# RapidAI/RapidDoc

Measured on AMD Instinct MI355X. Metric: pages/sec (layout+OCR det/rec), higher is better.
Workload: dtype f32

## Files before the change

### include/rapiddoc_mi355.h

```cpp
#ifndef RAPIDDOC_MI355_H
#define RAPIDDOC_MI355_H

#include <stddef.h>
#include <stdint.h>

#ifdef __cplusplus
extern "C" {
#endif

typedef struct rd_handle rd_handle;

#define RD_REC_UNFUSED_CTC 1
#define RD_REC_WANT_SOFTMAX 2
#define RD_REC_WANT_LOGITS 4
#define RD_REC_WANT_NECK 64

const char* rd_version(void);
rd_handle* rd_create(int device_id, const char* model_kind);
const char* rd_create_error(void);
void rd_destroy(rd_handle* h);
const char* rd_last_error(rd_handle* h);

int rd_load_weights(rd_handle* h, const void* safetensors_image, size_t nbytes);

int rd_query_workspace(rd_handle* h, int B, int H, int W, int flags, size_t* ws_bytes);

int rd_det_forward(rd_handle* h, const float* x_nchw_dev, int B, int H, int W, float* prob_b1hw_dev, void* ws_dev,
                   size_t ws_bytes, void* stream);
#define RD_DET_WANT_NECK 1
int rd_det_forward_ex(rd_handle* h, const float* x_nchw_dev, int B, int H, int W, float* prob_b1hw_dev, int flags, float* aux_dev,
                      void* ws_dev, size_t ws_bytes, void* stream);

int rd_rec_forward(rd_handle* h, const float* x_nchw_dev, int B, int W, int32_t* idx_bt_dev, float* prob_bt_dev,
                   float* full_btc_dev, int flags, void* ws_dev, size_t ws_bytes, void* stream);
int rd_rec_num_classes(rd_handle* h);
#define RD_REC_STAGE_BACKBONE 8
#define RD_REC_STAGE_TAIL 16
int rd_rec_token_dim(rd_handle* h);
int rd_rec_backbone_forward(rd_handle* h, const float* x_nchw_dev, int B, int W, float* tokens_btd_dev, void* ws_dev, size_t ws_bytes,
                            void* stream);
int rd_rec_tail_forward(rd_handle* h, const float* tokens_dev, int n_tokens, int n_lines, int max_tokens, const int32_t* seg_dev,
                        const int32_t* tokinfo_dev, int32_t* idx_dev, float* prob_dev, void* ws_dev, size_t ws_bytes, void* stream);
#define RD_REC_LINE_WIDTHS 32
int rd_rec_backbone_forward_lines(rd_handle* h, const float* x_nchw_dev, int B, int W, const int32_t* line_tab_dev, float* tokens_dev,
                                  void* ws_dev, size_t ws_bytes, void* stream);
int rd_rec_seq_len(int W);

int rd_backbone_forward(rd_handle* h, const float* x_nchw_dev, int B, int H, int W, float* const feats_dev[4],
                        void* ws_dev, size_t ws_bytes, void* stream);

int rd_formula_encoder_forward(rd_handle* h, const float* x_nchw_dev, int B, int C, int H, int W, float* enc_dev,
                               void* ws_dev, size_t ws_bytes, void* stream);

int rd_formula_decode(rd_handle* h, const float* enc_dev, int B, int S, int max_new_tokens, int64_t* ids_dev, int32_t* n_cols,
                      void* stream);
int rd_formula_max_new_tokens(rd_handle* h);

int rd_preproc_resize_norm(int device_id, const uint8_t* hwc_u8_dev, int H, int W, int OH, int OW, const float mean[3],
                           const float std[3], float scale, int interp, int swap_rb, float* out_chw_dev, void* stream);

int rd_preproc_resize_norm_batch(int device_id, const uint8_t* pages_u8_dev, int P, int H, int W, int OH, int OW, const float mean[3],
                                 const float std[3], float scale, int interp, int swap_rb, float* out_nchw_dev, void* stream);

#define RD_RESIZE_AA_MAX_SIDE 16384
int rd_preproc_resize_aa_norm(int device_id, const uint8_t* hwc_u8_dev, int H, int W, int OH, int OW, const float mean[3],
                              const float std[3], int swap_rb, float* out_chw_dev, uint8_t* out_u8_hwc_dev, void* stream);

typedef struct rd_crop_desc {
    int32_t page;
    int32_t out_w;
    float crop_w, crop_h;
    float m[9];
    int32_t rot90;
    int32_t pad_;
} rd_crop_desc;
int rd_crop_resize_norm_batch(int device_id, const uint8_t* pages_u8_dev, int P, int H, int W,
                              const rd_crop_desc* descs_dev, int n, int out_h, int out_w_padded, const float mean[3],
                              const float std[3], float scale, int swap_rb, float* out_nchw_dev, void* stream);

typedef struct rd_line_crop_desc {
    int32_t page;
    int32_t out_w;
    int32_t crop_w, crop_h;
    int32_t rot90;
    int32_t scratch_off;
    double m[9];
} rd_line_crop_desc;
int rd_line_crops_batch(int device_id, const uint8_t* pages_u8_dev, int P, int H, int W, const rd_line_crop_desc* descs_dev,
                        int n, int64_t max_crop_pixels, uint8_t* scratch_u8_dev, int out_h, int out_w_padded, int swap_rb,
                        float* out_nchw_dev, void* stream);

int rd_line_warp_batch(int device_id, const uint8_t* pages_u8_dev, int P, int H, int W, const rd_line_crop_desc* descs_dev, int n,
                       int64_t max_crop_pixels, uint8_t* scratch_u8_dev, void* stream);
int rd_line_resize_norm_batch(int device_id, const rd_line_crop_desc* descs_dev, int n, const uint8_t* scratch_u8_dev, int out_h,
                              int out_w_padded, int swap_rb, float* out_nchw_dev, void* stream);

#define RD_CLS_WANT_AUX 1
int rd_cls_forward(rd_handle* h, const float* x_nchw_dev, int B, int H, int W, float* prob_b2_dev, int flags, float* aux_dev, void* ws_dev,
                   size_t ws_bytes, void* stream);
int rd_table_encoder_forward(rd_handle* h, const float* x_nchw_dev, int B, int H, int W, float* memory_bt768_dev, void* ws_dev, size_t ws_bytes,
                             void* stream);
typedef struct {
    int32_t prefix_id, eos_id, pad_id, bbox_close_id, bbox_first_id, bbox_last_id;
} rd_table_decode_cfg;
int rd_table_decode(rd_handle* h, const float* memory_dev, int B, int S, int max_new_tokens, const rd_table_decode_cfg* cfg, int64_t* ids_dev,
                    int32_t* n_tokens, void* stream);
int rd_line_flip180_batch(int device_id, const rd_line_crop_desc* descs_dev, int n, const float* cls_prob_n2_dev, float thresh,
                          uint8_t* scratch_u8_dev, int32_t* flipped_out_dev, void* stream);

int rd_ctc_collapse(int device_id, const int32_t* idx_bt_dev, const float* prob_bt_dev, int B, int T, const uint8_t* char_table_dev,
                    int max_len, int n_classes, uint8_t* out_dev, int row_bytes, void* stream);
int rd_ctc_collapse_lines(int device_id, const int32_t* idx_dev, const float* prob_dev, int n_lines, const int32_t* seg_dev, int max_tokens,
                          const uint8_t* char_table_dev, int max_len, int n_classes, uint8_t* out_dev, int row_bytes, uint16_t* kept_cols_dev,
                          float* kept_conf_dev, void* stream);
int rd_ctc_rows_text(const uint8_t* rows_host, int n, int row_bytes, uint8_t* text_out, int64_t text_cap, int64_t* byte_off_out,
                     int32_t* n_chars_out, double* conf_out, double* conf3_out);

typedef struct rd_text_box {
    float pts[8];
    float score;
} rd_text_box;
int rd_db_postprocess(const float* prob_host, int B, int H, int W, const int32_t* src_hw, float thresh, float box_thresh,
                      float unclip_ratio, int use_dilation, int max_candidates, rd_text_box* out, int max_out,
                      int32_t* n_out, int n_threads);

size_t rd_db_boxes_workspace(int B, int H, int W, int max_runs, int max_candidates);
int rd_db_boxes_device(int device_id, const float* prob_dev, int B, int H, int W, const int32_t* src_hw_dev, float thresh, float box_thresh,
                       float unclip_ratio, int use_dilation, int max_candidates, int max_runs, void* ws_dev, size_t ws_bytes,
                       rd_text_box* out_dev, int max_out, int32_t* n_out_dev, void* stream);

int rd_text_boxes_order_merge(const rd_text_box* boxes, const int32_t* counts, int B, int max_in, float* quads_out, int32_t* n_out);

typedef struct rd_layout_post_cfg {
    int32_t n_classes;
    int32_t image_index, formula_index;
    int32_t thresh_is_dict;
    const float* thresh;
    int32_t layout_nms;
    int32_t merge_kind;
    const int8_t* merge_per_class;
    int32_t unclip_kind;
    const float* unclip;
    const uint8_t* unclip_present;
} rd_layout_post_cfg;
int rd_layout_postprocess(const float* boxes, int n, int ncol, int img_w, int img_h, const rd_layout_post_cfg* cfg,
                          float* out, int32_t* out_order, int32_t* n_out);
int rd_layout_postprocess_select(const float* boxes, int n, int ncol, int img_w, int img_h, const rd_layout_post_cfg* cfg,
                                 float* sel_boxes, int32_t* sel_src, int32_t* n_sel);

int rd_msdeform_attn(int device_id, const float* value, const int32_t* shapes, const int32_t* level_start, const float* loc, const float* attn,
                     float* out, int B, int S, int H, int D, int Q, int L, int P, void* stream);
int rd_topk_rows(int device_id, const float* scores, int rows, int n, int k, float* out_vals, int32_t* out_idx, void* stream);
size_t rd_encoder_layer_workspace(int M, int Dm, int F);
int rd_encoder_layer(int device_id, const float* x, const float* pos, int B, int T, int Dm, int heads, int F, int act, const float* in_w,
                     const float* in_b, const float* out_w, const float* out_b, const float* ln1_g, const float* ln1_b, const float* w1,
                     const float* b1, const float* w2, const float* b2, const float* ln2_g, const float* ln2_b, float eps, float* out, void* ws,
                     size_t ws_bytes, void* stream);

int rd_find_external_contours(const uint8_t* mask, int h, int w, int32_t* pts_out, int max_pts, int32_t* counts_out, int max_contours,
                              int32_t* n_contours, int32_t* n_pts);
double rd_contour_area(const int32_t* pts, int n);
double rd_arc_length(const int32_t* pts, int n, int closed);
int rd_approx_poly_dp(const int32_t* pts, int n, double epsilon, int closed, int32_t* out, int32_t* n_out);
int rd_min_area_rect_points(const float* pts, int n, float* out8);
double rd_polygon_area(const double* a, int na);
double rd_polygon_intersection_area(const double* a, int na, const double* b, int nb);
int rd_fill_poly(uint8_t* img, int h, int w, const int32_t* pts, int n, int value);

double rd_rec_chunk_cost(int n_lines, int wpad, int n_cu);
int rd_rec_plan_chunks(const int32_t* wpad_sorted, int n, int n_min, int n_max, int n_step, int n_cu, int32_t* sizes_out, int max_out,
                       int32_t* n_out);
int rd_rec_plan_lines(const double* ratios, const int64_t* order, int n, int rec_batch_num, int img_h, int img_w, int launch_multiple,
                      int n_min, int n_max, int n_step, int n_cu, int64_t* line_w_out, double* line_ratio_out, int32_t* sizes_out,
                      int32_t* launch_w_out, int max_out, int32_t* n_out);

int rd_set_precision(rd_handle* h, const char* mode);
int rd_range_status(rd_handle* h, void* stream);

int rd_plan_stats(rd_handle* h, uint64_t* plans_built, uint64_t* graph_captures, uint64_t* graph_replays);

int rd_set_profiling(rd_handle* h, int on);
const char* rd_profile_json(rd_handle* h);

#ifdef __cplusplus
}
#endif
#endif
```

### rapiddoc_amd/_lib.py

```python
from __future__ import annotations

import ctypes as C
from pathlib import Path

_PKG = Path(__file__).resolve().parent
LIB_PATH = _PKG / "librapiddoc_mi355.so"
_lib = None

SYMBOLS = {
    "rd_version": (C.c_char_p, []),
    "rd_create": (C.c_void_p, [C.c_int, C.c_char_p]),
    "rd_create_error": (C.c_char_p, []),
    "rd_destroy": (None, [C.c_void_p]),
    "rd_last_error": (C.c_char_p, [C.c_void_p]),
    "rd_load_weights": (C.c_int, [C.c_void_p, C.c_void_p, C.c_size_t]),
    "rd_query_workspace": (C.c_int, [C.c_void_p, C.c_int, C.c_int, C.c_int, C.c_int, C.POINTER(C.c_size_t)]),
    "rd_det_forward": (C.c_int, [C.c_void_p, C.c_void_p, C.c_int, C.c_int, C.c_int, C.c_void_p, C.c_void_p, C.c_size_t, C.c_void_p]),
    "rd_det_forward_ex": (C.c_int, [C.c_void_p, C.c_void_p, C.c_int, C.c_int, C.c_int, C.c_void_p, C.c_int, C.c_void_p, C.c_void_p, C.c_size_t, C.c_void_p]),
    "rd_rec_forward": (C.c_int, [C.c_void_p, C.c_void_p, C.c_int, C.c_int, C.c_void_p, C.c_void_p, C.c_void_p, C.c_int, C.c_void_p, C.c_size_t, C.c_void_p]),
    "rd_rec_num_classes": (C.c_int, [C.c_void_p]),
    "rd_rec_token_dim": (C.c_int, [C.c_void_p]),
    "rd_rec_backbone_forward": (C.c_int, [C.c_void_p, C.c_void_p, C.c_int, C.c_int, C.c_void_p, C.c_void_p, C.c_size_t, C.c_void_p]),
    "rd_rec_backbone_forward_lines": (C.c_int, [C.c_void_p, C.c_void_p, C.c_int, C.c_int, C.c_void_p, C.c_void_p, C.c_void_p, C.c_size_t, C.c_void_p]),
    "rd_rec_tail_forward": (C.c_int, [C.c_void_p, C.c_void_p, C.c_int, C.c_int, C.c_int, C.c_void_p, C.c_void_p, C.c_void_p, C.c_void_p,
                                      C.c_void_p, C.c_size_t, C.c_void_p]),
    "rd_rec_seq_len": (C.c_int, [C.c_int]),
    "rd_backbone_forward": (C.c_int, [C.c_void_p, C.c_void_p, C.c_int, C.c_int, C.c_int, C.POINTER(C.c_void_p), C.c_void_p, C.c_size_t, C.c_void_p]),
    "rd_formula_encoder_forward": (C.c_int, [C.c_void_p, C.c_void_p, C.c_int, C.c_int, C.c_int, C.c_int, C.c_void_p, C.c_void_p, C.c_size_t, C.c_void_p]),
    "rd_formula_decode": (C.c_int, [C.c_void_p, C.c_void_p, C.c_int, C.c_int, C.c_int, C.c_void_p, C.POINTER(C.c_int32), C.c_void_p]),
    "rd_formula_max_new_tokens": (C.c_int, [C.c_void_p]),
    "rd_preproc_resize_norm": (C.c_int, [C.c_int, C.c_void_p, C.c_int, C.c_int, C.c_int, C.c_int, C.POINTER(C.c_float), C.POINTER(C.c_float), C.c_float, C.c_int, C.c_int, C.c_void_p, C.c_void_p]),
    "rd_preproc_resize_norm_batch": (C.c_int, [C.c_int, C.c_void_p, C.c_int, C.c_int, C.c_int, C.c_int, C.c_int, C.POINTER(C.c_float), C.POINTER(C.c_float), C.c_float, C.c_int, C.c_int, C.c_void_p, C.c_void_p]),
    "rd_preproc_resize_aa_norm": (C.c_int, [C.c_int, C.c_void_p, C.c_int, C.c_int, C.c_int, C.c_int, C.POINTER(C.c_float), C.POINTER(C.c_float), C.c_int, C.c_void_p, C.c_void_p, C.c_void_p]),
    "rd_crop_resize_norm_batch": (C.c_int, [C.c_int, C.c_void_p, C.c_int, C.c_int, C.c_int, C.c_void_p, C.c_int, C.c_int, C.c_int, C.POINTER(C.c_float), C.POINTER(C.c_float), C.c_float, C.c_int, C.c_void_p, C.c_void_p]),
    "rd_line_crops_batch": (C.c_int, [C.c_int, C.c_void_p, C.c_int, C.c_int, C.c_int, C.c_void_p, C.c_int, C.c_int64, C.c_void_p, C.c_int, C.c_int, C.c_int, C.c_void_p, C.c_void_p]),
    "rd_line_warp_batch": (C.c_int, [C.c_int, C.c_void_p, C.c_int, C.c_int, C.c_int, C.c_void_p, C.c_int, C.c_int64, C.c_void_p, C.c_void_p]),
    "rd_line_resize_norm_batch": (C.c_int, [C.c_int, C.c_void_p, C.c_int, C.c_void_p, C.c_int, C.c_int, C.c_int, C.c_void_p, C.c_void_p]),
    "rd_cls_forward": (C.c_int, [C.c_void_p, C.c_void_p, C.c_int, C.c_int, C.c_int, C.c_void_p, C.c_int, C.c_void_p, C.c_void_p, C.c_size_t, C.c_void_p]),
    "rd_table_encoder_forward": (C.c_int, [C.c_void_p, C.c_void_p, C.c_int, C.c_int, C.c_int, C.c_void_p, C.c_void_p, C.c_size_t, C.c_void_p]),
    "rd_table_decode": (C.c_int, [C.c_void_p, C.c_void_p, C.c_int, C.c_int, C.c_int, C.c_void_p, C.c_void_p, C.c_void_p, C.c_void_p]),
    "rd_line_flip180_batch": (C.c_int, [C.c_int, C.c_void_p, C.c_int, C.c_void_p, C.c_float, C.c_void_p, C.c_void_p, C.c_void_p]),
    "rd_ctc_collapse": (C.c_int, [C.c_int, C.c_void_p, C.c_void_p, C.c_int, C.c_int, C.c_void_p, C.c_int, C.c_int, C.c_void_p, C.c_int, C.c_void_p]),
    "rd_ctc_collapse_lines": (C.c_int, [C.c_int, C.c_void_p, C.c_void_p, C.c_int, C.c_void_p, C.c_int, C.c_void_p, C.c_int, C.c_int, C.c_void_p, C.c_int, C.c_void_p, C.c_void_p,
                                        C.c_void_p]),
    "rd_db_postprocess": (C.c_int, [C.c_void_p, C.c_int, C.c_int, C.c_int, C.c_void_p, C.c_float, C.c_float, C.c_float, C.c_int, C.c_int, C.c_void_p, C.c_int, C.c_void_p, C.c_int]),
    "rd_db_boxes_workspace": (C.c_size_t, [C.c_int, C.c_int, C.c_int, C.c_int, C.c_int]),
    "rd_db_boxes_device": (C.c_int, [C.c_int, C.c_void_p, C.c_int, C.c_int, C.c_int, C.c_void_p, C.c_float, C.c_float, C.c_float, C.c_int, C.c_int,
                                     C.c_int, C.c_void_p, C.c_size_t, C.c_void_p, C.c_int, C.c_void_p, C.c_void_p]),
    "rd_rec_chunk_cost": (C.c_double, [C.c_int, C.c_int, C.c_int]),
    "rd_rec_plan_chunks": (C.c_int, [C.c_void_p, C.c_int, C.c_int, C.c_int, C.c_int, C.c_int, C.c_void_p, C.c_int, C.c_void_p]),
    "rd_rec_plan_lines": (C.c_int, [C.c_void_p, C.c_void_p] + [C.c_int] * 9 + [C.c_void_p] * 4 + [C.c_int, C.c_void_p]),
    "rd_text_boxes_order_merge": (C.c_int, [C.c_void_p, C.c_void_p, C.c_int, C.c_int, C.c_void_p, C.c_void_p]),
    "rd_ctc_rows_text": (C.c_int, [C.c_void_p, C.c_int, C.c_int, C.c_void_p, C.c_int64, C.c_void_p, C.c_void_p, C.c_void_p, C.c_void_p]),
    "rd_layout_postprocess": (C.c_int, [C.c_void_p, C.c_int, C.c_int, C.c_int, C.c_int, C.c_void_p, C.c_void_p, C.c_void_p, C.c_void_p]),
    "rd_layout_postprocess_select": (C.c_int, [C.c_void_p, C.c_int, C.c_int, C.c_int, C.c_int, C.c_void_p, C.c_void_p, C.c_void_p, C.c_void_p]),
    "rd_find_external_contours": (C.c_int, [C.c_void_p, C.c_int, C.c_int, C.c_void_p, C.c_int, C.c_void_p, C.c_int, C.c_void_p, C.c_void_p]),
    "rd_contour_area": (C.c_double, [C.c_void_p, C.c_int]),
    "rd_arc_length": (C.c_double, [C.c_void_p, C.c_int, C.c_int]),
    "rd_approx_poly_dp": (C.c_int, [C.c_void_p, C.c_int, C.c_double, C.c_int, C.c_void_p, C.c_void_p]),
    "rd_min_area_rect_points": (C.c_int, [C.c_void_p, C.c_int, C.c_void_p]),
    "rd_polygon_area": (C.c_double, [C.c_void_p, C.c_int]),
    "rd_polygon_intersection_area": (C.c_double, [C.c_void_p, C.c_int, C.c_void_p, C.c_int]),
    "rd_fill_poly": (C.c_int, [C.c_void_p, C.c_int, C.c_int, C.c_void_p, C.c_int, C.c_int]),
    "rd_msdeform_attn": (C.c_int, [C.c_int] + [C.c_void_p] * 6 + [C.c_int] * 7 + [C.c_void_p]),
    "rd_topk_rows": (C.c_int, [C.c_int, C.c_void_p, C.c_int, C.c_int, C.c_int, C.c_void_p, C.c_void_p, C.c_void_p]),
    "rd_encoder_layer_workspace": (C.c_size_t, [C.c_int, C.c_int, C.c_int]),
    "rd_encoder_layer": (C.c_int, [C.c_int, C.c_void_p, C.c_void_p] + [C.c_int] * 6 + [C.c_void_p] * 12 + [C.c_float, C.c_void_p, C.c_void_p, C.c_size_t, C.c_void_p]),
    "rd_set_precision": (C.c_int, [C.c_void_p, C.c_char_p]),
    "rd_range_status": (C.c_int, [C.c_void_p, C.c_void_p]),
    "rd_plan_stats": (C.c_int, [C.c_void_p, C.POINTER(C.c_uint64), C.POINTER(C.c_uint64), C.POINTER(C.c_uint64)]),
    "rd_set_profiling": (C.c_int, [C.c_void_p, C.c_int]),
    "rd_profile_json": (C.c_char_p, [C.c_void_p]),
}

_I, _P, _F = C.c_int, C.c_void_p, C.c_float
DEBUG_SYMBOLS = {
    "rd_debug_det_forward_stages": (_I, [_P, _P, _I, _I, _I, _P, _P, _P]),
    "rd_debug_cls_forward_stages": (_I, [_P, _P, _I, _I, _I, _P, _P, _P, _P]),
    "rd_debug_table_decode": (_I, [_P, _P, _I, _I, _I, _P] + [_P] * 7),
    "rd_debug_table_encoder_taps": (_I, [_P, _P, _I, _I, _I, _P, _P, _P]),
    "rd_debug_formula_decode": (_I, [_P, _P, _I, _I, _I, _P, C.POINTER(C.c_int32), _P, _P, _P]),
    "rd_debug_resize_aa_coeffs": (_I, [_I, _I, _P, _P, C.c_int64]),
    "rd_debug_time_mixer": (_F, [_I] * 4 + [_P] * 6),
    "rd_debug_time_gemm": (_F, [_I] * 5 + [_P] * 6),
    "rd_debug_gemm_h1": (_F, [_I] * 5 + [_P, _I, _P, _P, _P, _I, _P, _I, _P]),
    "rd_debug_seqconv": (_F, [_I] * 8 + [_P, _I, _P, _I, _P, _P, _P, _P, _I, _P]),
    "rd_debug_det_local": (_F, [_I] * 5 + [_P] * 5 + [_F, _P, C.POINTER(C.c_int)]),
    "rd_debug_conv": (_F, [_I] * 14 + [_P] * 8),
    "rd_debug_stem34": (_F, [_I] * 11 + [_P] * 7),
    "rd_debug_dwconv": (_F, [_I] * 8 + [_P] * 8),
    "rd_debug_lcv3_dw": (_F, [_I] * 9 + [_P] * 8),
    "rd_debug_dw5_strip": (_F, [_I] * 11 + [_P] * 7),
    "rd_debug_mv1e_pool": (_I, [_I] * 4 + [_P] * 3),
    "rd_debug_derived_tensor": (C.c_long, [C.c_char_p, C.c_char_p, C.c_size_t, C.c_char_p, _P, C.c_long]),
    "rd_debug_mbv3_dw": (_F, [_I] * 12 + [_P] * 4),
    "rd_debug_mbv3_block": (_F, [_I] * 14 + [_P] * 8),
    "rd_debug_mbv3_block_ok": (_I, [_I] * 12),
    "rd_debug_mbv3s_dw": (_F, [_I] * 13 + [_P] * 4),
    "rd_debug_mbv3s_block": (_F, [_I] * 15 + [_P] * 12),
    "rd_debug_lcv3_dw_det": (_F, [_I] * 10 + [_P] * 5),
    "rd_debug_lcv3_block": (_F, [_I] * 9 + [_P] * 9),
    "rd_debug_time_ctc": (_F, [_I] * 4 + [_P] * 7 + [_I, _P]),
    "rd_debug_attention": (_I, [_I] * 4 + [_F, _P, _P, _P, _I, _P]),
    "rd_debug_vit_attention": (_I, [_I] * 4 + [_F, _P, _P]),
    "rd_debug_attention_limits": (_I, [_I, _P, _P]),
    "rd_debug_layernorm": (_I, [_I, _I, _P, _I, _P, _I, _P, _P, _F]),
    "rd_debug_ctc_head": (_I, [_I] * 3 + [_P, _I] + [_P] * 6 + [_I, _P, _P]),
    "rd_debug_dec_gemv": (_I, [_I] * 4 + [_P] * 7),
    "rd_debug_dec_attention": (_I, [_I] * 4 + [_P, _P, _I, C.c_longlong] + [_P] * 5 + [_P, _I, _P, _P, _I, _P, _I]),
    "rd_debug_dec_select": (_I, [_I, _P, _I, _I, _I, _P, _I, _P, _I, _I] + [_P] * 6),
}


class NativeLibraryError(RuntimeError):
    pass


def load():
    global _lib
    if _lib is not None:
        return _lib
    if not LIB_PATH.exists():
        raise NativeLibraryError(
            f"{LIB_PATH} is missing - build it with `python -m rapiddoc_amd.build` (hipcc, gfx950). "
            "rapiddoc_amd has no CPU fallback.")
    import torch
    lib = C.CDLL(str(LIB_PATH))
    for name, (res, args) in {**SYMBOLS, **DEBUG_SYMBOLS}.items():
        fn = getattr(lib, name)
        fn.restype = res
        fn.argtypes = args
    _lib = lib
    return lib
```

### rapiddoc_amd/build.py

```python
from __future__ import annotations

import os
import shutil
import subprocess
import sys
from concurrent.futures import ThreadPoolExecutor
from pathlib import Path

PKG = Path(__file__).resolve().parent
CSRC = PKG / "csrc"
OUT = PKG / "librapiddoc_mi355.so"
SOURCES = ["kernels_conv.hip", "kernels_conv_h3.hip", "kernels_conv_direct_h3.hip", "kernels_conv3x3_h1.hip", "kernels_conv9x9_h1.hip", "kernels_stem34.hip", "kernels_rtdetr.hip", "kernels_conv_stream_h3.hip", "kernels_gemm_h3_dma.hip", "kernels_gemm_h1.hip", "kernels_misc.hip", "kernels_dw_lds.hip", "kernels_stem_fused.hip", "kernels_image.hip", "kernels_resize_aa.hip", "kernels_dbpost.hip", "kernels_attention_h3.hip", "kernels_seqconv.hip", "kernels_det_local.hip", "kernels_lcv3.hip", "kernels_lcv3_det.hip", "kernels_mv1e.hip", "kernels_mbv3.hip", "kernels_mbv3s.hip", "kernels_vit_attn.hip", "kernels_lcv3_block.hip", "kernels_ctc.hip", "kernels_mixer.hip", "kernels_mixer_h3.hip", "kernels_mixer_ws.hip", "kernels_mixer_res.hip", "formula_decoder.hip", "table_decoder.hip", "engine.cpp", "builder.cpp", "builder_mobile.cpp", "models.cpp", "api.cpp", "api_debug.cpp", "db_postprocess.cpp", "layout_postprocess.cpp", "polygon_ops.cpp", "rec_chunks.cpp", "host_stages.cpp"]
FLAGS = ["--offload-arch=gfx950", "-O3", "-std=c++17", "-fPIC", "-Wall", "-Wno-unused-function", "-x", "hip"]
FILE_FLAGS = {"kernels_mixer_ws.hip": ["-fno-slp-vectorize", "-DRD_GELU_SCALAR"], "kernels_gemm_h1.hip": ["-fno-slp-vectorize"],
              "kernels_stem_fused.hip": ["-fno-slp-vectorize"]}


def extra_flags_for(src: str) -> list:
    return list(FILE_FLAGS.get(Path(src).name, []))


def _hipcc() -> str:
    for cand in (os.environ.get("HIPCC"), shutil.which("hipcc"), "/opt/rocm/bin/hipcc"):
        if cand and Path(cand).exists():
            return cand
    raise RuntimeError("hipcc not found (ROCm 7.x required)")


def needs_build() -> bool:
    if not OUT.exists():
        return True
    t = OUT.stat().st_mtime
    deps = list(CSRC.glob("*")) + [PKG.parent / "include" / "rapiddoc_mi355.h", Path(__file__)]
    return any(d.stat().st_mtime > t for d in deps)


def build(force: bool = False, verbose: bool = True, extra_flags: tuple = (), out: Path = None) -> Path:
    variant = out is not None
    if not variant and not force and not needs_build():
        return OUT
    hipcc = _hipcc()
    objdir = PKG / "build" / (Path(out).stem if variant else "")
    objdir.mkdir(parents=True, exist_ok=True)
    OUT_ = Path(out) if variant else OUT

    def compile_one(src: str) -> Path:
        obj = objdir / (src + ".o")
        cmd = [hipcc, *FLAGS, *extra_flags_for(src), *extra_flags, "-c", str(CSRC / src), "-o", str(obj)]
        r = subprocess.run(cmd, capture_output=True, text=True)
        if r.returncode != 0:
            raise RuntimeError(f"hipcc failed for {src}:\n{r.stdout}\n{r.stderr}")
        if verbose and r.stderr.strip():
            print(r.stderr, file=sys.stderr)
        return obj

    with ThreadPoolExecutor(max_workers=min(8, len(SOURCES))) as ex:
        objs = list(ex.map(compile_one, SOURCES))
    tmp = OUT_.with_name(OUT_.name + f".tmp{os.getpid()}")
    cmd = [hipcc, "--offload-arch=gfx950", "-shared", "-fPIC", *map(str, objs), "-o", str(tmp)]
    r = subprocess.run(cmd, capture_output=True, text=True)
    if r.returncode != 0:
        tmp.unlink(missing_ok=True)
        raise RuntimeError(f"link failed:\n{r.stdout}\n{r.stderr}")
    os.replace(tmp, OUT_)
    if verbose:
        print(f"built {OUT_} ({OUT_.stat().st_size/1e6:.1f} MB)")
    return OUT_


if __name__ == "__main__":
    build(force="--force" in sys.argv)
```

### rapiddoc_amd/csrc/api.cpp

```cpp
#include <algorithm>
#include <mutex>
#include <string>

#include "api_handle.h"

static thread_local std::string g_create_err;

static bool is_family(const rd_handle* h, rd::ModelFamily f) { return h->eng && h->eng->model().family == f; }
static bool is_rec(const rd_handle* h) { return is_family(h, rd::ModelFamily::Recogniser); }
static bool is_det(const rd_handle* h) { return is_family(h, rd::ModelFamily::Detector); }

extern "C" {

const char* rd_version(void) { return "rapiddoc_mi355 0.3 (gfx950; fp32 results, split-fp16 + fp32 MFMA kernels)"; }

rd_handle* rd_create(int device_id, const char* model_kind) {
    try {
        if (!model_kind) throw rd::Error("model_kind is NULL");
        auto* h = new rd_handle();
        h->device = device_id;
        h->kind = model_kind;
        if (h->kind == "ppformulanet_head" || h->kind == "unitable_decoder") {
            int count = 0;
            if (hipGetDeviceCount(&count) != hipSuccess || count <= 0 || device_id < 0 || device_id >= count) {
                delete h;
                throw rd::Error("no HIP device available (MI355X required; there is no CPU fallback)");
            }
        } else {
            h->eng = new rd::Engine(device_id, model_kind);
        }
        g_create_err.clear();
        return h;
    } catch (const std::exception& e) {
        g_create_err = e.what();
        return nullptr;
    }
}
const char* rd_create_error(void) { return g_create_err.c_str(); }

void rd_destroy(rd_handle* h) {
    if (!h) return;
    delete h->eng;
    if (h->dec) rd::formula_decoder_destroy(h->dec);
    if (h->tdec) rd::table_decoder_destroy(h->tdec);
    delete h;
}
const char* rd_last_error(rd_handle* h) { return h ? h->err.c_str() : "null handle"; }

int rd_load_weights(rd_handle* h, const void* img, size_t nbytes) {
    return guarded(h, [&] {
        if (h->kind == "ppformulanet_head") {
            RD_CHECK(!h->dec, "weights already loaded for this handle");
            h->dec = rd::formula_decoder_create(h->device, img, nbytes);
        } else if (h->kind == "unitable_decoder") {
            RD_CHECK(!h->tdec, "weights already loaded for this handle");
            h->tdec = rd::table_decoder_create(h->device, img, nbytes);
        } else {
            h->eng->load_weights(img, nbytes);
        }
    });
}

int rd_query_workspace(rd_handle* h, int B, int H, int W, int flags, size_t* ws_bytes) {
    return guarded(h, [&] {
        RD_CHECK(ws_bytes, "ws_bytes is NULL");
        RD_CHECK(h->eng, "this model kind owns its workspace");
        if (is_rec(h) && !(flags & rd::REC_STAGE_TAIL)) H = 48;
        *ws_bytes = h->eng->workspace_bytes(B, H, W, flags);
    });
}

int rd_det_forward(rd_handle* h, const float* x, int B, int H, int W, float* prob, void* ws, size_t ws_bytes, void* stream) {
    return guarded(h, [&] {
        RD_CHECK(is_det(h), "handle is not a detector (ppocrv6_det / ppocrv5_det_server / ppocrv5_det_mobile / ppocrv3_det_mobile) model");
        RD_CHECK(x && prob && B > 0, "null input/output");
        h->eng->run(B, H, W, 0, {(void*)x, (void*)prob}, ws, ws_bytes, (hipStream_t)stream);
    });
}

int rd_det_forward_ex(rd_handle* h, const float* x, int B, int H, int W, float* prob, int flags, float* aux, void* ws, size_t ws_bytes,
                      void* stream) {
    return guarded(h, [&] {
        RD_CHECK(is_det(h), "handle is not a detector (ppocrv6_det / ppocrv5_det_server / ppocrv5_det_mobile / ppocrv3_det_mobile) model");
        RD_CHECK(x && prob && B > 0, "null input/output");
        RD_CHECK((flags & ~RD_DET_WANT_NECK) == 0, "rd_det_forward_ex: unknown flag");
        if (flags & RD_DET_WANT_NECK) {
            RD_CHECK(h->eng->model().det_want_neck,
                     "RD_DET_WANT_NECK is offered by ppocrv5_det_server, ppocrv5_det_mobile and ppocrv3_det_mobile only");
            RD_CHECK(aux, "aux_dev is NULL");
        }
        h->eng->run(B, H, W, flags, {(void*)x, (void*)prob, (void*)aux}, ws, ws_bytes, (hipStream_t)stream);
    });
}

int rd_cls_forward(rd_handle* h, const float* x, int B, int H, int W, float* prob, int flags, float* aux, void* ws, size_t ws_bytes, void* stream) {
    return guarded(h, [&] {
        RD_CHECK(h->eng && h->eng->kind() == "ppocr_cls_mobile", "handle is not a text-line classifier (ppocr_cls_mobile) model");
        RD_CHECK(x && prob && B > 0, "null input/output");
        RD_CHECK((flags & ~RD_CLS_WANT_AUX) == 0, "rd_cls_forward: unknown flag");
        RD_CHECK(!(flags & RD_CLS_WANT_AUX) || aux, "aux_dev is NULL");
        h->eng->run(B, H, W, flags, {(void*)x, (void*)prob, (void*)aux}, ws, ws_bytes, (hipStream_t)stream);
    });
}

int rd_table_encoder_forward(rd_handle* h, const float* x, int B, int H, int W, float* memory, void* ws, size_t ws_bytes, void* stream) {
    return guarded(h, [&] {
        RD_CHECK(h->eng && h->eng->kind() == "unitable_encoder", "handle is not a table-structure encoder (unitable_encoder) model");
        RD_CHECK(x && memory && B > 0, "null input/output");
        h->eng->run(B, H, W, 0, {(void*)x, (void*)memory}, ws, ws_bytes, (hipStream_t)stream);
    });
}


int rd_table_decode(rd_handle* h, const float* memory, int B, int S, int max_new_tokens, const rd_table_decode_cfg* cfg, int64_t* ids, int32_t* n_tokens,
                    void* stream) {
    return guarded(h, [&] {
        RD_CHECK(h->kind == "unitable_decoder" && h->tdec, "handle is not a loaded table-structure decoder (unitable_decoder)");
        int c[6];
        table_cfg6(cfg, c);
        rd::table_decoder_decode(h->tdec, memory, B, S, max_new_tokens, c, (long long*)ids, (int*)n_tokens, (hipStream_t)stream, nullptr, nullptr, nullptr,
                                 nullptr, nullptr);
    });
}

int rd_line_flip180_batch(int device_id, const rd_line_crop_desc* descs, int n, const float* cls_prob, float thresh, uint8_t* scratch,
                          int32_t* flipped_out, void* stream) {
    if (!descs || !cls_prob || !scratch || !flipped_out || n < 0) return 1;
    if (hipSetDevice(device_id) != hipSuccess) return 1;
    if (rd::launch_line_flip180(reinterpret_cast<const rd::LineCropDesc*>(descs), n, cls_prob, thresh, scratch, flipped_out, (hipStream_t)stream) != 0) return 1;
    return hipGetLastError() == hipSuccess ? 0 : 1;
}

int rd_rec_forward(rd_handle* h, const float* x, int B, int W, int32_t* idx, float* prob, float* full, int flags, void* ws,
                   size_t ws_bytes, void* stream) {
    return guarded(h, [&] {
        RD_CHECK(is_rec(h), "handle is not a recogniser (ppocrv6_rec / ppocrv5_rec_server / ppocrv5_rec_mobile / ppocr_rec_mv1e) model");
        RD_CHECK(x && idx && prob && B > 0, "null input/output");
        if (flags & (RD_REC_WANT_SOFTMAX | RD_REC_WANT_LOGITS | RD_REC_WANT_NECK)) RD_CHECK(full, "full_btc_dev is NULL");
        RD_CHECK(!((flags & RD_REC_WANT_SOFTMAX) && (flags & RD_REC_WANT_LOGITS)), "choose softmax OR logits");
        RD_CHECK(!(flags & RD_REC_WANT_NECK) || flags == RD_REC_WANT_NECK, "RD_REC_WANT_NECK goes with no other flag");
        h->eng->run(B, 48, W, flags, {(void*)x, (void*)idx, (void*)prob, (void*)full}, ws, ws_bytes, (hipStream_t)stream);
    });
}
int rd_rec_token_dim(rd_handle* h) { return (h && is_rec(h)) ? h->eng->rec_token_dim() : -1; }
int rd_rec_backbone_forward(rd_handle* h, const float* x, int B, int W, float* tokens, void* ws, size_t ws_bytes, void* stream) {
    return guarded(h, [&] {
        RD_CHECK(is_rec(h), "handle is not a recogniser (ppocrv6_rec / ppocrv5_rec_server / ppocrv5_rec_mobile / ppocr_rec_mv1e) model");
        RD_CHECK(x && tokens && B > 0, "null input/output");
        h->eng->run(B, 48, W, rd::REC_STAGE_BACKBONE, {(void*)x, (void*)tokens}, ws, ws_bytes, (hipStream_t)stream);
    });
}
int rd_rec_backbone_forward_lines(rd_handle* h, const float* x, int B, int W, const int32_t* line_tab, float* tokens, void* ws, size_t ws_bytes,
                                  void* stream) {
    return guarded(h, [&] {
        RD_CHECK(is_rec(h), "handle is not a ppocrv6_rec / ppocrv5_rec_mobile / ppocr_rec_mv1e model");
        RD_CHECK(h->eng->model().rec_line_widths, "rd_rec_backbone_forward_lines: per-line widths inside one backbone launch are out of scope for " +
                                                      h->eng->kind() + " (run the backbone stage once per padded width)");
        RD_CHECK(x && tokens && line_tab && B > 0, "null input/output");
        h->eng->run(B, 48, W, rd::REC_STAGE_BACKBONE | rd::REC_LINE_WIDTHS, {(void*)x, (void*)tokens, (void*)line_tab}, ws, ws_bytes,
                    (hipStream_t)stream);
    });
}
int rd_rec_tail_forward(rd_handle* h, const float* tokens, int n_tokens, int n_lines, int max_tokens, const int32_t* seg,
                        const int32_t* tokinfo, int32_t* idx, float* prob, void* ws, size_t ws_bytes, void* stream) {
    return guarded(h, [&] {
        RD_CHECK(is_rec(h), "handle is not a recogniser (ppocrv6_rec / ppocrv5_rec_server / ppocrv5_rec_mobile / ppocr_rec_mv1e) model");
        RD_CHECK(tokens && seg && tokinfo && idx && prob && n_tokens > 0 && n_lines > 0 && max_tokens > 0, "null input/output");
        h->eng->run(n_lines, max_tokens, n_tokens, rd::REC_STAGE_TAIL,
                    {(void*)tokens, (void*)idx, (void*)prob, nullptr, (void*)seg, (void*)tokinfo}, ws, ws_bytes, (hipStream_t)stream);
    });
}
int rd_rec_seq_len(int W) {
    if (W < 16) return 0;
    const int w1 = (W - 1) / 2 + 1, w2 = (w1 - 1) / 2 + 1;
    return (w2 - 2) / 2 + 1;
}
int rd_rec_num_classes(rd_handle* h) { return (h && h->eng) ? h->eng->n_classes() : -1; }

int rd_backbone_forward(rd_handle* h, const float* x, int B, int H, int W, float* const feats[4], void* ws, size_t ws_bytes,
                        void* stream) {
    return guarded(h, [&] {
        RD_CHECK(h->eng && h->eng->kind() == "pphgnetv2_b4", "handle is not a pphgnetv2_b4 model");
        RD_CHECK(x && feats && feats[0] && feats[1] && feats[2] && feats[3], "null input/output");
        h->eng->run(B, H, W, 0, {(void*)x, (void*)feats[0], (void*)feats[1], (void*)feats[2], (void*)feats[3]}, ws, ws_bytes,
                    (hipStream_t)stream);
    });
}

int rd_formula_encoder_forward(rd_handle* h, const float* x, int B, int C, int H, int W, float* enc, void* ws, size_t ws_bytes,
                               void* stream) {
    return guarded(h, [&] {
        RD_CHECK(h->eng && h->eng->kind() == "pphgnetv2_b6_formula", "handle is not a pphgnetv2_b6_formula model");
        RD_CHECK(x && enc && B > 0 && (C == 1 || C == 3), "null input/output or channel count not 1/3");
        h->eng->run(B, H, W, C == 1 ? 1 : 0, {(void*)x, (void*)enc}, ws, ws_bytes, (hipStream_t)stream);
    });
}

int rd_formula_decode(rd_handle* h, const float* enc, int B, int S, int max_new_tokens, int64_t* ids, int32_t* n_cols, void* stream) {
    return guarded(h, [&] {
        RD_CHECK(h->kind == "ppformulanet_head" && h->dec, "handle is not a loaded ppformulanet_head model");
        RD_CHECK(enc && ids && n_cols, "null input/output");
        *n_cols = rd::formula_decoder_decode(h->dec, enc, B, S, max_new_tokens, reinterpret_cast<long long*>(ids), (hipStream_t)stream, nullptr,
                                             nullptr);
    });
}
int rd_formula_max_new_tokens(rd_handle* h) { return (h && h->dec) ? rd::formula_decoder_max_new(h->dec) : -1; }

int rd_preproc_resize_norm(int device_id, const uint8_t* src, int H, int W, int OH, int OW, const float mean[3],
                           const float std[3], float scale, int interp, int swap_rb, float* out, void* stream) {
    if (!src || !out || H <= 0 || W <= 0 || OH <= 0 || OW <= 0 || (interp != 1 && interp != 2)) return 1;
    if (hipSetDevice(device_id) != hipSuccess) return 1;
    rd::PreprocParams p{};
    p.src = src; p.H = H; p.W = W; p.dst = out; p.OH = OH; p.OW = OW;
    for (int i = 0; i < 3; ++i) { p.mean[i] = mean ? mean[i] : 0.f; p.inv_std[i] = 1.f / (std ? std[i] : 1.f); }
    p.scale = scale; p.interp = interp; p.swap_rb = swap_rb;
    rd::launch_preproc_resize_norm(p, (hipStream_t)stream);
    return hipGetLastError() == hipSuccess ? 0 : 1;
}

int rd_preproc_resize_norm_batch(int device_id, const uint8_t* src, int P, int H, int W, int OH, int OW, const float mean[3],
                                 const float std[3], float scale, int interp, int swap_rb, float* out, void* stream) {
    if (!src || !out || P <= 0 || P > 65535 || H <= 0 || W <= 0 || OH <= 0 || OW <= 0 || (interp != 1 && interp != 2)) return 1;
    if (hipSetDevice(device_id) != hipSuccess) return 1;
    rd::PreprocParams p{};
    p.src = src; p.H = H; p.W = W; p.dst = out; p.OH = OH; p.OW = OW;
    for (int i = 0; i < 3; ++i) { p.mean[i] = mean ? mean[i] : 0.f; p.inv_std[i] = 1.f / (std ? std[i] : 1.f); }
    p.scale = scale; p.interp = interp; p.swap_rb = swap_rb;
    p.batch = P; p.src_stride = (size_t)H * W * 3; p.dst_stride = (size_t)3 * OH * OW;
    rd::launch_preproc_resize_norm(p, (hipStream_t)stream);
    return hipGetLastError() == hipSuccess ? 0 : 1;
}

int rd_preproc_resize_aa_norm(int device_id, const uint8_t* src, int H, int W, int OH, int OW, const float mean[3], const float std[3],
                              int swap_rb, float* out, uint8_t* out_u8, void* stream) {
    std::string err;
    const int rc = rd::launch_resize_aa_norm(device_id, src, H, W, OH, OW, mean, std, swap_rb, out, out_u8, (hipStream_t)stream, err);
    if (rc != 0) g_create_err = err;
    return rc;
}

int rd_crop_resize_norm_batch(int device_id, const uint8_t* pages, int P, int H, int W, const rd_crop_desc* descs, int n,
                              int out_h, int out_w_padded, const float mean[3], const float std[3], float scale, int swap_rb,
                              float* out, void* stream) {
    static_assert(sizeof(rd_crop_desc) == sizeof(rd::CropDesc), "rd_crop_desc layout");
    if (!pages || !descs || !out || P <= 0 || n < 0 || out_h <= 0 || out_w_padded <= 0) return 1;
    if (hipSetDevice(device_id) != hipSuccess) return 1;
    rd::CropBatchParams p{};
    p.pages = pages; p.H = H; p.W = W; p.page_stride = (size_t)H * W * 3;
    p.descs = reinterpret_cast<const rd::CropDesc*>(descs); p.n = n;
    p.dst = out; p.OH = out_h; p.OWp = out_w_padded;
    for (int i = 0; i < 3; ++i) { p.mean[i] = mean ? mean[i] : 0.f; p.inv_std[i] = 1.f / (std ? std[i] : 1.f); }
    p.scale = scale; p.swap_rb = swap_rb;
    rd::launch_crop_resize_norm_batch(p, (hipStream_t)stream);
    return hipGetLastError() == hipSuccess ? 0 : 1;
}

int rd_line_crops_batch(int device_id, const uint8_t* pages, int P, int H, int W, const rd_line_crop_desc* descs, int n,
                        int64_t max_crop_pixels, uint8_t* scratch, int out_h, int out_w_padded, int swap_rb, float* out, void* stream) {
    static_assert(sizeof(rd_line_crop_desc) == sizeof(rd::LineCropDesc), "rd_line_crop_desc layout");
    if (!pages || !descs || !out || !scratch || P <= 0 || n < 0 || out_h <= 0 || out_w_padded <= 0 || max_crop_pixels <= 0) return 1;
    if (hipSetDevice(device_id) != hipSuccess) return 1;
    rd::LineCropParams p{};
    p.pages = pages; p.H = H; p.W = W; p.page_stride = (size_t)H * W * 3;
    p.descs = reinterpret_cast<const rd::LineCropDesc*>(descs); p.n = n;
    p.scratch = scratch; p.max_crop_pixels = (long)max_crop_pixels;
    p.dst = out; p.OH = out_h; p.OWp = out_w_padded; p.swap_rb = swap_rb;
    if (rd::launch_line_crops(p, (hipStream_t)stream) != 0) return 1;
    return hipGetLastError() == hipSuccess ? 0 : 1;
}

int rd_line_warp_batch(int device_id, const uint8_t* pages, int P, int H, int W, const rd_line_crop_desc* descs, int n,
                       int64_t max_crop_pixels, uint8_t* scratch, void* stream) {
    if (!pages || !descs || !scratch || P <= 0 || n < 0 || max_crop_pixels <= 0) return 1;
    if (hipSetDevice(device_id) != hipSuccess) return 1;
    rd::LineCropParams p{};
    p.pages = pages; p.H = H; p.W = W; p.page_stride = (size_t)H * W * 3;
    p.descs = reinterpret_cast<const rd::LineCropDesc*>(descs); p.n = n;
    p.scratch = scratch; p.max_crop_pixels = (long)max_crop_pixels;
    if (rd::launch_line_warp(p, (hipStream_t)stream) != 0) return 1;
    return hipGetLastError() == hipSuccess ? 0 : 1;
}
int rd_line_resize_norm_batch(int device_id, const rd_line_crop_desc* descs, int n, const uint8_t* scratch, int out_h, int out_w_padded,
                              int swap_rb, float* out, void* stream) {
    if (!descs || !scratch || !out || n < 0 || out_h <= 0 || out_w_padded <= 0) return 1;
    if (hipSetDevice(device_id) != hipSuccess) return 1;
    rd::LineCropParams p{};
    p.descs = reinterpret_cast<const rd::LineCropDesc*>(descs); p.n = n;
    p.scratch = const_cast<uint8_t*>(scratch);
    p.dst = out; p.OH = out_h; p.OWp = out_w_padded; p.swap_rb = swap_rb;
    if (rd::launch_line_resize_norm(p, (hipStream_t)stream) != 0) return 1;
    return hipGetLastError() == hipSuccess ? 0 : 1;
}

int rd_ctc_collapse(int device_id, const int32_t* idx, const float* prob, int B, int T, const uint8_t* ctab, int max_len, int n_classes,
                    uint8_t* out, int row_bytes, void* stream) {
    if (!idx || !prob || !ctab || !out || B < 0 || T <= 0 || max_len <= 0 || n_classes <= 0) return 1;
    if (hipSetDevice(device_id) != hipSuccess) return 1;
    if (rd::launch_ctc_collapse(idx, prob, B, T, nullptr, ctab, max_len, n_classes, out, row_bytes, nullptr, nullptr, (hipStream_t)stream) != 0) return 1;
    return hipGetLastError() == hipSuccess ? 0 : 1;
}

int rd_ctc_collapse_lines(int device_id, const int32_t* idx, const float* prob, int n_lines, const int32_t* seg, int max_tokens,
                          const uint8_t* ctab, int max_len, int n_classes, uint8_t* out, int row_bytes, uint16_t* kept_cols, float* kept_conf,
                          void* stream) {
    if (!idx || !prob || !seg || !ctab || !out || n_lines < 0 || max_tokens <= 0 || max_len <= 0 || n_classes <= 0) return 1;
    if (hipSetDevice(device_id) != hipSuccess) return 1;
    if (rd::launch_ctc_collapse(idx, prob, n_lines, max_tokens, seg, ctab, max_len, n_classes, out, row_bytes, kept_cols, kept_conf,
                                (hipStream_t)stream) != 0)
        return 1;
    return hipGetLastError() == hipSuccess ? 0 : 1;
}

int rd_msdeform_attn(int device_id, const float* value, const int32_t* shapes, const int32_t* level_start, const float* loc, const float* attn,
                     float* out, int B, int S, int H, int D, int Q, int L, int P, void* stream) {
    if (!value || !shapes || !level_start || !loc || !attn || !out || B < 0 || S <= 0 || H <= 0 || D <= 0 || Q < 0 || L <= 0 || P <= 0 || H * D > 1024)
        return 1;
    if (hipSetDevice(device_id) != hipSuccess) return 1;
    rd::launch_msdeform_attn(value, shapes, level_start, loc, attn, out, B, S, H, D, Q, L, P, (hipStream_t)stream);
    return hipGetLastError() == hipSuccess ? 0 : 1;
}

int rd_topk_rows(int device_id, const float* scores, int rows, int n, int k, float* out_vals, int32_t* out_idx, void* stream) {
    if (!scores || !out_vals || !out_idx || rows < 0 || n <= 0 || k <= 0 || k > 1024 || k > n) return 1;
    if (hipSetDevice(device_id) != hipSuccess) return 1;
    rd::launch_topk_rows(scores, rows, n, k, out_vals, out_idx, (hipStream_t)stream);
    return hipGetLastError() == hipSuccess ? 0 : 1;
}

size_t rd_encoder_layer_workspace(int M, int Dm, int F) {
    if (M <= 0 || Dm <= 0 || F <= 0) return 0;
    return ((size_t)M * Dm * 3  + (size_t)M * 3 * Dm  + (size_t)M * F) * sizeof(float);
}

int rd_encoder_layer(int device_id, const float* x, const float* pos, int B, int T, int Dm, int heads, int F, int act, const float* in_w,
                     const float* in_b, const float* out_w, const float* out_b, const float* ln1_g, const float* ln1_b, const float* w1,
                     const float* b1, const float* w2, const float* b2, const float* ln2_g, const float* ln2_b, float eps, float* out, void* ws,
                     size_t ws_bytes, void* stream) {
    const int M = B * T;
    if (!x || !in_w || !out_w || !w1 || !w2 || !ln1_g || !ln1_b || !ln2_g || !ln2_b || !out || !ws || B <= 0 || T <= 0 || heads <= 0 ||
        Dm % heads != 0 || Dm % 4 != 0 || F % 4 != 0 || ws_bytes < rd_encoder_layer_workspace(M, Dm, F))
        return 1;
    const int hd = Dm / heads;
    if (hd != 16 && hd != 32) return 1;
    if (hipSetDevice(device_id) != hipSuccess) return 1;
    hipStream_t s = (hipStream_t)stream;
    float* xp = (float*)ws;
    float* att = xp + (size_t)M * Dm;
    float* y1 = att + (size_t)M * Dm;
    float* qkv = y1 + (size_t)M * Dm;
    float* ff = qkv + (size_t)M * 3 * Dm;
    auto gemm = [&](const float* a, int K, const float* w, const float* b, int N, float* y, int yld, int a_act, const float* res) {
        rd::ConvParams p{};
        p.x = a; p.xld = K; p.N = 1; p.H = 1; p.W = M; p.Cin = K;
        p.w = w; p.bias = b; p.y = y; p.yld = yld; p.OH = 1; p.OW = M; p.Cout = N;
        p.KH = p.KW = p.SH = p.SW = 1;
        p.res = res; p.rld = N;
        p.act = a_act; p.out_mode = rd::OUT_NHWC;
        p.M = M; p.K = K; p.Ng = N;
        rd::launch_conv_igemm(p, s);
    };
    try {
        const float* qk_in = x;
        if (pos) {
            rd::launch_add(x, Dm, pos, Dm, xp, Dm, M, Dm, s);
            qk_in = xp;
        }
        gemm(qk_in, Dm, in_w, in_b, 2 * Dm, qkv, 3 * Dm, rd::ACT_NONE, nullptr);
        gemm(x, Dm, in_w + (size_t)2 * Dm * Dm, in_b ? in_b + 2 * Dm : nullptr, Dm, qkv + 2 * Dm, 3 * Dm, rd::ACT_NONE, nullptr);
        rd::launch_attention(qkv, att, B, T, heads, hd, 1.0f / std::sqrt((float)hd), s);
        gemm(att, Dm, out_w, out_b, Dm, xp, Dm, rd::ACT_NONE, x);
        rd::launch_layernorm(xp, Dm, y1, Dm, ln1_g, ln1_b, M, Dm, eps, s);
        gemm(y1, Dm, w1, b1, F, ff, F, act, nullptr);
        gemm(ff, F, w2, b2, Dm, xp, Dm, rd::ACT_NONE, y1);
        rd::launch_layernorm(xp, Dm, out, Dm, ln2_g, ln2_b, M, Dm, eps, s);
    } catch (...) {
        return 1;
    }
    return hipGetLastError() == hipSuccess ? 0 : 1;
}

size_t rd_db_boxes_workspace(int B, int H, int W, int max_runs, int max_candidates) {
    (void)W;
    if (B <= 0 || H <= 0 || max_runs <= 0 || max_candidates <= 0) return 0;
    return rd::db_boxes_workspace_bytes(B, H, max_runs, max_candidates);
}
int rd_db_boxes_device(int device_id, const float* prob, int B, int H, int W, const int32_t* src_hw_dev, float thresh, float box_thresh,
                       float unclip_ratio, int use_dilation, int max_candidates, int max_runs, void* ws, size_t ws_bytes, rd_text_box* out,
                       int max_out, int32_t* n_out, void* stream) {
    if (!prob || !src_hw_dev || !ws || !out || !n_out || B < 0 || H <= 0 || W <= 0) return 1;
    if (hipSetDevice(device_id) != hipSuccess) return 1;
    if (rd::launch_db_boxes(prob, B, H, W, src_hw_dev, thresh, box_thresh, unclip_ratio, use_dilation, max_candidates, max_runs, ws, ws_bytes,
                            out, max_out, n_out, (hipStream_t)stream) != 0)
        return 1;
    return hipGetLastError() == hipSuccess ? 0 : 1;
}

int rd_set_precision(rd_handle* h, const char* mode) {
    return guarded(h, [&] {
        RD_CHECK(h->eng, "precision modes apply to the network engines");
        const std::string m = mode ? mode : "";
        RD_CHECK(m == "auto" || m == "fp32" || m == "h3", "precision must be auto, fp32 or h3");
        h->eng->set_precision(m == "h3" ? rd::Engine::PREC_H3 : m == "fp32" ? rd::Engine::PREC_FP32 : rd::Engine::PREC_AUTO);
    });
}
int rd_range_status(rd_handle* h, void* stream) {
    int out = 0;
    const int rc = guarded(h, [&] { if (h->eng) out = h->eng->take_range_flag((hipStream_t)stream); });
    return rc != 0 ? -1 : out;
}

int rd_plan_stats(rd_handle* h, uint64_t* plans_built, uint64_t* graph_captures, uint64_t* graph_replays) {
    if (!h || !h->eng) return 1;
    if (plans_built) *plans_built = h->eng->plans_built();
    if (graph_captures) *graph_captures = h->eng->graph_captures();
    if (graph_replays) *graph_replays = h->eng->graph_replays();
    return 0;
}

int rd_set_profiling(rd_handle* h, int on) {
    return guarded(h, [&] { if (h->eng) h->eng->set_profiling(on != 0); });
}
const char* rd_profile_json(rd_handle* h) {
    if (!h || !h->eng) return "[]";
    h->prof = h->eng->profile_json();
    return h->prof.c_str();
}

}
```

### rapiddoc_amd/csrc/host_stages.cpp

```cpp
#include <algorithm>
#include <charconv>
#include <cstdint>
#include <cstring>
#include <vector>

#include "../../include/rapiddoc_mi355.h"

#pragma clang fp contract(off)

namespace {

struct Quad {
    float p[8];
};
struct BBox {
    float x0, y0, x1, y1;
};

bool quad_is_tilted(const Quad& q) {
    const float height = ((q.p[7] - q.p[1]) + (q.p[5] - q.p[3])) / 2.0f;
    const float diag = q.p[5] - q.p[1];
    return !(0.8f * height <= diag && diag <= 1.2f * height);
}

bool y_overlap_exceeds(const BBox& a, const BBox& b, float thr) {
    const float d = std::min(a.y1, b.y1) - std::max(a.y0, b.y0);
    const float ov = d > 0.0f ? d : 0.0f;
    const float mh = std::min(a.y1 - a.y0, b.y1 - b.y0);
    return mh > 0.0f ? (ov / mh) > thr : false;
}

void put_bbox(const BBox& b, float* o) {
    o[0] = b.x0; o[1] = b.y0; o[2] = b.x1; o[3] = b.y0; o[4] = b.x1; o[5] = b.y1; o[6] = b.x0; o[7] = b.y1;
}

int order_merge_page(const rd_text_box* in, int k, float* out) {
    std::vector<Quad> q((size_t)k);
    for (int i = 0; i < k; ++i)
        for (int c = 0; c < 8; ++c) q[i].p[c] = (float)(int32_t)in[i].pts[c];
    std::stable_sort(q.begin(), q.end(), [](const Quad& a, const Quad& b) { return a.p[1] < b.p[1] || (a.p[1] == b.p[1] && a.p[0] < b.p[0]); });
    for (int i = 0; i + 1 < k; ++i)
        for (int j = i; j >= 0; --j) {
            const float dy = q[j + 1].p[1] - q[j].p[1];
            if ((dy < 0.0f ? -dy : dy) < 10.0f && q[j + 1].p[0] < q[j].p[0]) std::swap(q[j], q[j + 1]);
            else break;
        }
    std::vector<BBox> flat;
    std::vector<int> tilted;
    flat.reserve((size_t)k);
    for (int i = 0; i < k; ++i) {
        if (quad_is_tilted(q[i])) tilted.push_back(i);
        else flat.push_back({q[i].p[0], q[i].p[1], q[i].p[2], q[i].p[5]});
    }
    std::stable_sort(flat.begin(), flat.end(), [](const BBox& a, const BBox& b) { return a.y0 < b.y0; });
    int n = 0;
    std::vector<BBox> line, merged;
    const size_t nf = flat.size();
    for (size_t lo = 0; lo < nf;) {
        size_t hi = lo + 1;
        while (hi < nf && y_overlap_exceeds(flat[hi], flat[hi - 1], 0.6f)) ++hi;
        float x_min = flat[lo].x0, x_max = flat[lo].x1, y_min = flat[lo].y0, y_max = flat[lo].y1;
        for (size_t i = lo + 1; i < hi; ++i) {
            x_min = std::min(x_min, flat[i].x0); x_max = std::max(x_max, flat[i].x1);
            y_min = std::min(y_min, flat[i].y0); y_max = std::max(y_max, flat[i].y1);
        }
        if (x_max - x_min > (y_max - y_min) * 4.0f) {
            line.assign(flat.begin() + lo, flat.begin() + hi);
            std::stable_sort(line.begin(), line.end(), [](const BBox& a, const BBox& b) { return a.x0 < b.x0; });
            merged.clear();
            for (BBox b : line) {
                if (!merged.empty() && !(merged.back().x1 < b.x0)) {
                    const BBox m = merged.back();
                    merged.pop_back();
                    b = {std::min(m.x0, b.x0), std::min(m.y0, b.y0), std::max(m.x1, b.x1), std::max(m.y1, b.y1)};
                }
                merged.push_back(b);
            }
            for (const BBox& m : merged) put_bbox(m, out + 8 * (size_t)n++);
        } else {
            for (size_t i = lo; i < hi; ++i) put_bbox(flat[i], out + 8 * (size_t)n++);
        }
        lo = hi;
    }
    for (int i : tilted) std::memcpy(out + 8 * (size_t)n++, q[i].p, sizeof(q[i].p));
    return n;
}

}

extern "C" int rd_text_boxes_order_merge(const rd_text_box* boxes, const int32_t* counts, int B, int max_in, float* quads_out, int32_t* n_out) {
    if (B < 0 || max_in < 0 || (B > 0 && (!boxes || !counts || !quads_out || !n_out))) return 1;
    for (int b = 0; b < B; ++b)
        if (counts[b] < 0 || counts[b] > max_in) return 1;
    for (int b = 0; b < B; ++b)
        n_out[b] = order_merge_page(boxes + (size_t)b * max_in, counts[b], quads_out + (size_t)b * max_in * 8);
    return 0;
}

extern "C" int rd_ctc_rows_text(const uint8_t* rows, int n, int row_bytes, uint8_t* text_out, int64_t text_cap, int64_t* byte_off_out,
                                int32_t* n_chars_out, double* conf_out, double* conf3_out) {
    if (n < 0 || row_bytes < 16 || text_cap < 0 || !byte_off_out || (n > 0 && (!rows || !n_chars_out || !conf_out || !conf3_out))) return 1;
    int64_t pos = 0;
    byte_off_out[0] = 0;
    for (int b = 0; b < n; ++b) {
        const uint8_t* row = rows + (size_t)b * row_bytes;
        int32_t nbytes;
        float conf;
        std::memcpy(&nbytes, row, 4);
        std::memcpy(&conf, row + 4, 4);
        if (nbytes < 0 || nbytes > row_bytes - 16) return 1;
        if (pos + nbytes > text_cap || (nbytes > 0 && !text_out)) return 2;
        int32_t chars = 0;
        for (int32_t i = 0; i < nbytes; ++i) {
            const uint8_t c = row[16 + i];
            text_out[pos + i] = c;
            chars += (c & 0xC0) != 0x80;
        }
        pos += nbytes;
        byte_off_out[b + 1] = pos;
        n_chars_out[b] = chars;
        const double s = (double)conf;
        conf_out[b] = s;
        char buf[400];
        const auto w = std::to_chars(buf, buf + sizeof(buf), s, std::chars_format::fixed, 3);
        double r = s;
        if (w.ec == std::errc()) std::from_chars(buf, w.ptr, r);
        conf3_out[b] = r;
    }
    return 0;
}
```

### rapiddoc_amd/pipeline.py

```python
from __future__ import annotations

import os
import time
import ctypes as C
from concurrent.futures import ThreadPoolExecutor
from dataclasses import dataclass, field
from typing import Dict, List, Optional, Sequence, Tuple

import numpy as np
import torch

from . import _lib, ocr_host
from .engine import RdEngine, preproc_resize_norm, preproc_resize_norm_batch
from .rec_plan import (CLS_IMG_H, CLS_IMG_W, LINE_DTYPE, RecPlan, plan_rec,
                       quad_to_crop_matrix, quads_to_crop_matrices)

LAYOUT_SIZE = 800
DET_LIMIT = 960


class CropDesc(C.Structure):
    _fields_ = [("page", C.c_int32), ("out_w", C.c_int32), ("crop_w", C.c_float), ("crop_h", C.c_float),
                ("m", C.c_float * 9), ("rot90", C.c_int32), ("pad_", C.c_int32)]


def cls_flip_rule(prob: np.ndarray, thresh: float) -> np.ndarray:
    p = np.asarray(prob, dtype=np.float32).reshape(-1, 2)
    return (p[:, 1] > p[:, 0]) & (p[:, 1] >= np.float32(thresh))


def flip180(crop: np.ndarray) -> np.ndarray:
    return np.ascontiguousarray(np.asarray(crop)[::-1, ::-1])


CROP_DTYPE = np.dtype([("page", "<i4"), ("out_w", "<i4"), ("crop_w", "<f4"), ("crop_h", "<f4"), ("m", "<f4", (9,)),
                       ("rot90", "<i4"), ("pad_", "<i4")])
assert CROP_DTYPE.itemsize == C.sizeof(CropDesc)


def boxes_to_quads(boxes_xyxy: np.ndarray) -> np.ndarray:
    b = np.asarray(boxes_xyxy, dtype=np.float32).reshape(-1, 4)
    return np.stack([b[:, [0, 1]], b[:, [2, 1]], b[:, [2, 3]], b[:, [0, 3]]], axis=1)


@dataclass
class PageResult:
    lines: List[Tuple[np.ndarray, str, float]] = field(default_factory=list)
    layout_feats: Optional[List[torch.Tensor]] = None
    cls: Optional[List[Tuple[bool, int, float]]] = None


@dataclass(slots=True)
class _RecLaunch:
    x: Optional[torch.Tensor] = None
    event: Optional[torch.cuda.Event] = None
    done: Optional[torch.cuda.Event] = None
    idx: Optional[torch.Tensor] = None
    prob: Optional[torch.Tensor] = None
    rows: Optional[torch.Tensor] = None
    cols: Optional[Tuple[torch.Tensor, torch.Tensor]] = None
    cls_prob: Optional[torch.Tensor] = None
    cls_flip: Optional[torch.Tensor] = None


class PagePipeline:
    def __init__(self, states: Dict[str, object], device: int = 0, characters: Optional[Sequence[str]] = None,
                 rec_batch_num: Optional[int] = None, rec_width_multiple: int = 32, keep_feats: bool = False, n_rec_streams: int = 4,
                 rec_mode: Optional[str] = None, rec_chunking: Optional[str] = None, use_cls: bool = False, cls_thresh: float = 0.9):
        self.use_cls, self.cls_thresh = bool(use_cls), float(cls_thresh)
        if self.use_cls and "ppocr_cls_mobile" not in states:
            raise ValueError("use_cls=True needs the text-line classifier's weights: states['ppocr_cls_mobile'] (ch_ptocr_mobile_v2.0_cls_mobile)")
        if rec_mode is None:
            rec_mode = "strict" if rec_batch_num is None and rec_chunking is None else "throughput"
        if rec_mode not in ("strict", "throughput"):
            raise ValueError("rec_mode must be 'strict' or 'throughput'")
        if rec_chunking is None:
            rec_chunking = "adaptive" if rec_batch_num is None else "fixed"
        if rec_batch_num is None:
            rec_batch_num = 64
        if rec_chunking not in ("fixed", "adaptive"):
            raise ValueError("rec_chunking must be 'fixed' or 'adaptive'")
        self.rec_mode = rec_mode
        self.rec_chunking = rec_chunking
        if rec_mode == "strict":
            rec_batch_num, rec_width_multiple = 6, 1
        self.device = device
        self.tdev = torch.device("cuda", device)
        self.n_cu = int(torch.cuda.get_device_properties(self.tdev).multi_processor_count)
        det_kinds = [k for k in ("ppocrv6_det", "ppocrv5_det_server", "ppocrv5_det_mobile", "ppocrv3_det_mobile") if k in states]
        if len(det_kinds) != 1:
            raise ValueError("states must carry exactly one detector: 'ppocrv6_det' or 'ppocrv5_det_server' or 'ppocrv5_det_mobile' or 'ppocrv3_det_mobile'")
        self.det_kind = det_kinds[0]
        self.det = RdEngine(self.det_kind, device, guard="deferred", reuse_outputs=True).load_weights(states[self.det_kind])
        rec_kinds = [k for k in ("ppocrv6_rec", "ppocrv5_rec_server", "ppocrv5_rec_mobile", "ppocr_rec_mv1e") if k in states]
        if len(rec_kinds) != 1:
            raise ValueError("states must carry exactly one recogniser: 'ppocrv6_rec' or 'ppocrv5_rec_server' or 'ppocrv5_rec_mobile' or 'ppocr_rec_mv1e'")
        self.rec_kind = rec_kinds[0]
        self.rec_lines_in_launch = self.rec_kind in ("ppocrv6_rec", "ppocrv5_rec_mobile", "ppocr_rec_mv1e")
        self.rec_engines = [RdEngine(self.rec_kind, device, guard="deferred").load_weights(states[self.rec_kind]) for _ in range(max(1, n_rec_streams))]
        self.rec = self.rec_engines[0]
        self.rec_streams = [torch.cuda.Stream(device=self.tdev) for _ in self.rec_engines]
        self.rec_tail = RdEngine(self.rec_kind, device, guard="deferred").load_weights(states[self.rec_kind])
        self.cls_engines = ([RdEngine("ppocr_cls_mobile", device, guard="deferred").load_weights(states["ppocr_cls_mobile"]) for _ in self.rec_engines]
                            if self.use_cls else [])
        self.last_cls = None
        self.tail_stream = torch.cuda.Stream(device=self.tdev)
        self.layout_stream = torch.cuda.Stream(device=self.tdev)
        self.front_stream = torch.cuda.Stream(device=self.tdev)
        self._prefetched: Optional[dict] = None
        self._after_rec_enqueue = None
        self.prefetch_gate = float(os.environ.get("RD_PREFETCH_GATE", "1.0"))
        self.layout = RdEngine("pphgnetv2_b4", device, guard="deferred", reuse_outputs=True).load_weights(states["pphgnetv2_b4"]) if "pphgnetv2_b4" in states else None
        self._bufs: Dict[tuple, torch.Tensor] = {}
        ncls = self.rec.num_classes
        self.characters = list(characters) if characters is not None else ["blank"] + [chr(0x4E00 + i) for i in range(ncls - 2)] + [" "]
        assert len(self.characters) == ncls, (len(self.characters), ncls)
        self.rec_batch_num = rec_batch_num
        self.rec_width_multiple = rec_width_multiple
        self.keep_feats = keep_feats
        tab, self._ctc_max_len = ocr_host.char_table(self.characters)
        self._ctc_table = torch.from_numpy(tab).to(self.tdev)
        self.device_ctc = True
        self.device_db = True
        self.host_native = ocr_host.host_native_default()
        self.db_ws: dict = {}
        self.rec_two_stage = os.environ.get("RD_REC_TWO_STAGE", "1") != "0"
        self.rec_width_sync = None
        self._sync_this_call = True
        self._width_sync_cache = None
        self._width_sync_epoch, self._in_run_batch = 0, False
        self.keep_rec_inputs = False
        self.last_rec_batches: List[Tuple[np.ndarray, torch.Tensor, torch.Tensor, torch.Tensor]] = []
        self._lib = _lib.load()
        self.stats: Dict[str, float] = {}

    def _buf(self, role, numel: int, dtype=torch.float32) -> torch.Tensor:
        key = (role, dtype)
        t = self._bufs.get(key)
        if t is None or t.numel() < numel:
            t = self._bufs[key] = torch.empty(int(numel * 1.25) + 64, dtype=dtype, device=self.tdev)
        return t[:numel]

    def layout_preprocess(self, pages: torch.Tensor) -> torch.Tensor:
        P = pages.shape[0]
        out = self._buf("layout_x", P * 3 * LAYOUT_SIZE * LAYOUT_SIZE).view(P, 3, LAYOUT_SIZE, LAYOUT_SIZE)
        return preproc_resize_norm_batch(pages, (LAYOUT_SIZE, LAYOUT_SIZE), interp=2, out=out)

    def layout_forward(self, pages: torch.Tensor) -> List[torch.Tensor]:
        return self.layout.backbone_forward(self.layout_preprocess(pages))

    def det_preprocess(self, pages: torch.Tensor) -> Tuple[torch.Tensor, Tuple[int, int]]:
        P, H, W, _ = pages.shape
        bh, bw = -(-(H + 100) // 64) * 64, -(-(W + 100) // 64) * 64
        dh, dw = ocr_host.det_resize_shape(bh, bw, DET_LIMIT, "max")
        out = self._buf("det_x", P * 3 * dh * dw).view(P, 3, dh, dw)
        x = preproc_resize_norm_batch(pages, (dh, dw), mean=ocr_host.DET_MEAN, std=ocr_host.DET_STD, interp=1, swap_rb=True, out=out)
        return x, (dh, dw)

    def det_forward(self, pages: torch.Tensor) -> Tuple[torch.Tensor, Tuple[int, int]]:
        x, det_hw = self.det_preprocess(pages)
        return self.det.det_forward(x), det_hw

    def rec_forward_lines(self, pages: torch.Tensor, quads_per_page: Sequence[np.ndarray]):
        return self.rec_forward_sources([(pages, quads_per_page)])[0]

    def rec_forward_sources(self, sources: Sequence[Tuple[torch.Tensor, Sequence[np.ndarray]]],
                            image_keys: Optional[Sequence[Sequence[int]]] = None, want_words: bool = False,
                            pooled: bool = True):
        self._sync_this_call = bool(pooled)
        if not self._in_run_batch:
            self._width_sync_epoch += 1
        out = self._rec_forward_sources_once(sources, image_keys, want_words)
        for _ in range(3):
            if not any([e.check_range_and_fallback() for e in self.rec_engines + [self.rec_tail] + self.cls_engines]):
                break
            self.stats["range_fallbacks"] = self.stats.get("range_fallbacks", 0) + 1
            out = self._rec_forward_sources_once(sources, image_keys, want_words)
        return out

    def _synced_widths(self, sync, keys: np.ndarray, ratios: np.ndarray):
        sig = (self._width_sync_epoch, keys.tobytes(), ratios.tobytes())
        if self._width_sync_cache is not None and self._width_sync_cache[0] == sig:
            return self._width_sync_cache[1]
        res = sync(keys, ratios)
        self._width_sync_cache = (sig, res)
        return res

    def _collapse_home(self, name: str, n: int, T: int, call, *extra: torch.Tensor) -> List[torch.Tensor]:
        row_bytes = (16 + T * self._ctc_max_len + 15) // 16 * 16
        rows = torch.empty((n, row_bytes), dtype=torch.uint8, device=self.tdev)
        if call(rows.data_ptr(), row_bytes) != 0:
            raise RuntimeError(f"{name} failed")
        home = []
        for t in (rows,) + extra:
            h = torch.empty(t.shape, dtype=t.dtype, pin_memory=True)
            h.copy_(t, non_blocking=True)
            home.append(h)
        return home

    def _collapse_rows(self, idx: torch.Tensor, prob: torch.Tensor, nb: int, st, record: bool = True):
        rows = done = None
        with torch.cuda.stream(st):
            if self.device_ctc:
                T = idx.shape[1]
                rows, = self._collapse_home("rd_ctc_collapse", nb, T, lambda out, row_bytes: self._lib.rd_ctc_collapse(
                    self.device, idx.data_ptr(), prob.data_ptr(), nb, T, self._ctc_table.data_ptr(), self._ctc_max_len, len(self.characters),
                    out, row_bytes, st.cuda_stream))
            if record:
                done = torch.cuda.Event()
                done.record(st)
        return rows, done

    def _collapse_lines(self, idx_all: torch.Tensor, prob_all: torch.Tensor, tables: torch.Tensor, n_lines: int, max_tokens: int, st,
                        want_cols: bool = False):
        with torch.cuda.stream(st):
            cols = torch.empty((n_lines, max_tokens), dtype=torch.int16, device=self.tdev) if want_cols else None
            confs = torch.empty((n_lines, max_tokens), dtype=torch.float32, device=self.tdev) if want_cols else None
            rows, *cols_h = self._collapse_home("rd_ctc_collapse_lines", n_lines, max_tokens, lambda out, row_bytes: self._lib.rd_ctc_collapse_lines(
                self.device, idx_all.data_ptr(), prob_all.data_ptr(), n_lines, tables.data_ptr(), max_tokens, self._ctc_table.data_ptr(),
                self._ctc_max_len, len(self.characters), out, row_bytes, cols.data_ptr() if want_cols else None,
                confs.data_ptr() if want_cols else None, st.cuda_stream), *((cols, confs) if want_cols else ()))
            done = torch.cuda.Event()
            done.record(st)
        return rows, done, tuple(cols_h) if want_cols else None

    def _rec_forward_sources_once(self, sources, image_keys=None, want_words=False):
        t0 = time.perf_counter()
        if self.use_cls and want_words:
            raise ValueError("use_cls together with want_words: rapidocr defines no word-box mapping for lines turned by 180 degrees")
        self.last_cls = None
        for imgs, _quads in sources:
            assert imgs.is_cuda and imgs.dtype == torch.uint8 and imgs.dim() == 4 and imgs.is_contiguous()
        strict = self.rec_mode == "strict"
        sync = None
        if self.rec_width_sync is not None and strict and self.rec_two_stage and self._sync_this_call:
            sync = lambda keys, ratios: self._synced_widths(self.rec_width_sync, keys, ratios)
        plan = plan_rec([(imgs.shape[0], quads) for imgs, quads in sources], image_keys, strict=strict, two_stage=self.rec_two_stage,
                        lines_in_launch=self.rec_lines_in_launch, chunking=self.rec_chunking, rec_batch_num=self.rec_batch_num,
                        rec_width_multiple=self.rec_width_multiple, n_cu=self.n_cu, n_streams=len(self.rec_engines), use_cls=self.use_cls,
                        host_native=self.host_native, want_words=want_words, width_sync=sync)
        scatter = lambda per_line: self._scatter_texts(per_line, plan.src_of, plan.page_of, plan.n_img, plan.perm)
        cls_of: List[tuple] = [(False, 0, 0.0)] * plan.n_all
        if plan.n == 0:
            if self.use_cls and plan.n_all:
                self.last_cls = scatter(cls_of)
            return scatter([("", 0.0, None) if want_words else ("", 0.0)] * plan.n_all)
        if getattr(self, "_crop_scratch", None) is None or self._crop_scratch.numel() < plan.scratch_bytes:
            self._crop_scratch = torch.empty(int(plan.scratch_bytes * 1.25) + 1024, dtype=torch.uint8, device=sources[0][0].device)
        self.stats["t_descs_ms"] = (time.perf_counter() - t0) * 1e3
        main = torch.cuda.current_stream()
        launches = self._enqueue_rec(plan, sources, want_words)
        self.stats["t_rec_enqueue_ms"] = (time.perf_counter() - t0) * 1e3 - self.stats["t_descs_ms"]
        hook, self._after_rec_enqueue = self._after_rec_enqueue, None
        if hook is not None:
            t_h = time.perf_counter()
            S, nb = len(self.rec_engines), len(launches)
            m = max(1, min(nb, int(np.ceil(self.prefetch_gate * nb))))
            hook([l.event for l in launches[max(0, m - S): m]])
            self.stats["t_front_next_ms"] = (time.perf_counter() - t_h) * 1e3
        texts = self._decode_rec(plan, launches, want_words)
        for st in self.rec_streams + [self.tail_stream]:
            main.wait_stream(st)
        self.stats["rec_lines"] = plan.n
        self.stats["rec_batches"] = len(launches)
        self.last_pool_order = plan.perm
        if self.use_cls:
            ph = np.concatenate([l.cls_prob.numpy() for l in launches])
            fh = np.concatenate([l.cls_flip.numpy() for l in launches])
            for j, i in enumerate(plan.line_ids.tolist()):
                label = int(ph[j, 1] > ph[j, 0])
                cls_of[i] = (bool(fh[j]), label, float(ph[j, label]))
            self.last_cls = scatter(cls_of)
            self.last_cls_prob = (plan.line_ids, ph)
        return scatter(texts)

    def _enqueue_rec(self, plan: RecPlan, sources, want_words: bool) -> List[_RecLaunch]:
        dev, S, lib = sources[0][0].device, len(self.rec_engines), self._lib
        keep_inputs = self.keep_rec_inputs
        upload = lambda descs: torch.from_numpy(descs.view(np.uint8)).to(dev, non_blocking=True)
        descs_dev = upload(plan.descs)
        cls = None
        if self.use_cls:
            cls = (upload(plan.descs_cls), self._buf("cls_prob", 2 * plan.n).view(plan.n, 2), self._buf("cls_flip", plan.n, torch.int32),
                   torch.empty((plan.n, 2), dtype=torch.float32, pin_memory=True), torch.empty((plan.n,), dtype=torch.int32, pin_memory=True))
        descs_warp_dev = upload(plan.descs_warp) if plan.descs_warp is not None else descs_dev
        if keep_inputs:
            self.last_rec_descs = (plan.descs.copy(), np.asarray(plan.batch_base, dtype=np.int64), np.asarray(plan.starts, dtype=np.int64))
            self.last_cls_inputs = []
        main = torch.cuda.current_stream()
        ready = torch.cuda.Event()
        ready.record(main)
        tokens = linetab = tables = None
        if plan.two_stage:
            base = plan.group_base
            tokens = self._buf("rec_tokens", int(base[-1]) * self.rec.rec_token_dim).view(int(base[-1]), self.rec.rec_token_dim)
            for gi, lens in enumerate(plan.group_lens):
                tokens[int(base[gi]) + int(lens.sum()): int(base[gi + 1])].zero_()
            tables = [self.rec_tail.rec_tail_tables(lp, dev, out=self._buf(("tail_tab", gi), 2 * len(lp) + int(lp.sum()), torch.int32))
                      for gi, (lp, _t) in enumerate(plan.group_pad)]
            if plan.linetab is not None:
                tab_h = torch.from_numpy(plan.linetab).pin_memory()
                linetab = self._buf("rec_linetab", 4 * plan.n, torch.int32).view(plan.n, 4)
                linetab.copy_(tab_h, non_blocking=True)
                self._keep_linetab = tab_h
            ready.record(main)
            self.tail_stream.wait_event(ready)
        launches: List[_RecLaunch] = []
        for bi, (chunk, wpad) in enumerate(plan.batches):
            nb, pos = len(chunk), int(plan.starts[bi])
            k = bi % S
            st = self.rec_streams[k]
            if bi < S:
                st.wait_event(ready)
            with torch.cuda.stream(st):
                x = self._buf(("rec_x", k), nb * 3 * ocr_host.REC_IMG_H * wpad).view(nb, 3, ocr_host.REC_IMG_H, wpad)
                scratch = self._crop_scratch.data_ptr() + int(plan.batch_base[bi])
                for si, first, cnt, max_px in plan.warp_jobs[bi]:
                    imgs = sources[si][0]
                    rc = lib.rd_line_warp_batch(self.device, imgs.data_ptr(), imgs.shape[0], imgs.shape[1], imgs.shape[2],
                                                descs_warp_dev.data_ptr() + first * LINE_DTYPE.itemsize, cnt, max_px, scratch, st.cuda_stream)
                    if rc != 0:
                        raise RuntimeError("rd_line_warp_batch failed")
                launch = _RecLaunch()
                if cls is not None:
                    self._enqueue_cls(launch, cls, descs_dev, k, pos, nb, scratch, plan.line_ids[pos: pos + nb])
                rc = lib.rd_line_resize_norm_batch(self.device, descs_dev.data_ptr() + pos * LINE_DTYPE.itemsize, nb, scratch,
                                                   ocr_host.REC_IMG_H, wpad, 1, x.data_ptr(), st.cuda_stream)
                if rc != 0:
                    raise RuntimeError("rd_line_resize_norm_batch failed")
                if plan.lines_in_launch:
                    self.rec_engines[k].rec_backbone_forward_lines(x, linetab[pos: pos + nb], tokens)
                elif plan.two_stage:
                    self.rec_engines[k].rec_backbone_forward(x, tokens[plan.tok_lo[bi]: plan.tok_lo[bi] + nb * int(plan.seq_line[pos])])
                else:
                    launch.idx, launch.prob, _ = self.rec_engines[k].rec_forward(x)
                    launch.rows, launch.done = self._collapse_rows(launch.idx, launch.prob, nb, st)
                launch.event = launch.done
                if plan.two_stage:
                    launch.event = torch.cuda.Event()
                    launch.event.record(st)
                launch.x = x.clone() if keep_inputs else x
            launches.append(launch)
            if plan.two_stage and ((bi + 1) % S == 0 or bi + 1 == len(plan.batches)):
                self._enqueue_tail(plan, launches, bi // S, tokens, tables[bi // S], want_words)
        return launches

    def _enqueue_cls(self, launch: _RecLaunch, cls, descs_dev, k: int, pos: int, nb: int, scratch: int, line_ids: np.ndarray) -> None:
        descs_cls_dev, cls_prob, cls_flip, cls_prob_h, cls_flip_h = cls
        stream = torch.cuda.current_stream().cuda_stream
        sl = slice(pos, pos + nb)
        xc = self._buf(("cls_x", k), nb * 3 * CLS_IMG_H * CLS_IMG_W).view(nb, 3, CLS_IMG_H, CLS_IMG_W)
        rc = self._lib.rd_line_resize_norm_batch(self.device, descs_cls_dev.data_ptr() + pos * LINE_DTYPE.itemsize, nb, scratch,
                                                 CLS_IMG_H, CLS_IMG_W, 1, xc.data_ptr(), stream)
        if rc != 0:
            raise RuntimeError("rd_line_resize_norm_batch (classifier) failed")
        self.cls_engines[k].cls_forward(xc, out=cls_prob[sl])
        if self.keep_rec_inputs:
            self.last_cls_inputs.append((line_ids, xc.clone()))
        rc = self._lib.rd_line_flip180_batch(self.device, descs_dev.data_ptr() + pos * LINE_DTYPE.itemsize, nb, cls_prob[sl].data_ptr(),
                                             self.cls_thresh, scratch, cls_flip[sl].data_ptr(), stream)
        if rc != 0:
            raise RuntimeError("rd_line_flip180_batch failed")
        launch.cls_prob, launch.cls_flip = cls_prob_h[sl], cls_flip_h[sl]
        launch.cls_prob.copy_(cls_prob[sl], non_blocking=True)
        launch.cls_flip.copy_(cls_flip[sl], non_blocking=True)

    def _enqueue_tail(self, plan: RecPlan, launches: List[_RecLaunch], gi: int, tokens: torch.Tensor, tables: torch.Tensor, want_words: bool) -> None:
        grp = [launches[bi] for bi in plan.groups[gi]]
        t_lo, t_hi = int(plan.group_base[gi]), int(plan.group_base[gi + 1])
        lens_pad, max_tokens = plan.group_pad[gi]
        for launch in grp:
            self.tail_stream.wait_event(launch.event)
        with torch.cuda.stream(self.tail_stream):
            n_tok = t_hi - t_lo
            idx_all, prob_all = self.rec_tail.rec_tail_forward(
                tokens[t_lo:t_hi], lens_pad, tables, max_tokens=max_tokens,
                out=(self._buf(("tail_idx", gi), n_tok, torch.int32), self._buf(("tail_prob", gi), n_tok)))
        done = None
        if plan.lines_mode:
            last = grp[-1]
            last.rows, done, last.cols = self._collapse_lines(idx_all, prob_all, tables, len(plan.group_lens[gi]), max_tokens, self.tail_stream,
                                                              want_words)
            if self.keep_rec_inputs:
                with torch.cuda.stream(self.tail_stream):
                    last.idx, last.prob = idx_all.clone(), prob_all.clone()
        else:
            for bi, launch in zip(plan.groups[gi], grp):
                nb, t = len(plan.batches[bi][0]), int(plan.seq_line[int(plan.starts[bi])])
                lo = plan.tok_lo[bi] - t_lo
                launch.idx, launch.prob = idx_all[lo: lo + nb * t].view(nb, t), prob_all[lo: lo + nb * t].view(nb, t)
                launch.rows, ev = self._collapse_rows(launch.idx, launch.prob, nb, self.tail_stream, record=launch is grp[-1])
                done = ev or done
        for launch in grp:
            launch.done = done

    def _texts_from_rows(self, rows_np: np.ndarray, line_ids: np.ndarray, texts: list) -> None:
        if self.host_native:
            txt, _conf, conf3 = ocr_host.parse_ctc_rows_native(rows_np)
            for i, t, s in zip(line_ids.tolist(), txt, conf3):
                texts[i] = (t, s)
        else:
            for i, (t, s) in zip(line_ids.tolist(), ocr_host.parse_ctc_rows(rows_np)):
                texts[i] = (t, ocr_host.format_score(s))

    def _words_from_rows(self, plan: RecPlan, lo: int, rows_np: np.ndarray, cols, texts: list) -> None:
        n_kept = rows_np[:, 8:12].copy().view("<i4")[:, 0]
        cols_np, confs_np = cols[0].numpy(), cols[1].numpy()
        for j, (t, sc) in enumerate(ocr_host.parse_ctc_rows(rows_np)):
            i, k = int(plan.order_all[lo + j]), int(n_kept[j])
            words = {"cols": cols_np[j, :k].astype(np.int64).tolist(), "confs": confs_np[j, :k].astype(np.float64).tolist(),
                     "n_steps": int(plan.seq_line[lo + j]), "wh_ratio": float(plan.ratios[i]), "max_wh_ratio": float(plan.line_ratio[lo + j]),
                     "crop_hw": (int(plan.eff_h[i]), int(plan.eff_w[i]))}
            texts[int(plan.keep[i])] = (t, sc, words)

    def _decode_groups(self, plan: RecPlan, launches: List[_RecLaunch], want_words: bool, texts: list) -> list:
        ids, starts = plan.line_ids, plan.starts
        t_dec = 0.0
        for gi, grp in enumerate(plan.groups):
            tail = launches[grp[-1]]
            tail.done.synchronize()
            t1 = time.perf_counter()
            lo, hi = int(starts[grp[0]]), int(starts[grp[-1] + 1])
            if want_words:
                self._words_from_rows(plan, lo, tail.rows.numpy(), tail.cols, texts)
            else:
                self._texts_from_rows(tail.rows.numpy(), ids[lo:hi], texts)
            t_dec += time.perf_counter() - t1
            if tail.idx is not None:
                g0 = int(plan.group_base[gi])
                for bi in grp:
                    a, e = int(starts[bi]), int(starts[bi + 1])
                    sl = [(int(plan.first_tok[i]) - g0, int(plan.seq_line[i])) for i in range(a, e)]
                    self.last_rec_batches.append((ids[a:e], launches[bi].x, np.asarray(plan.line_w[a:e]),
                                                  [tail.idx[o: o + t] for o, t in sl], [tail.prob[o: o + t] for o, t in sl]))
        self.stats["t_decode_ms"] = t_dec * 1e3
        return texts

    def _decode_rec(self, plan: RecPlan, launches: List[_RecLaunch], want_words: bool) -> list:
        texts: List[tuple] = [("", 0.0, None) if want_words else ("", 0.0)] * plan.n_all
        ids, starts = plan.line_ids, plan.starts
        t_dec = 0.0
        if self.keep_rec_inputs:
            self.last_rec_crop_sizes = (plan.crop_w.astype(np.int64), plan.crop_h.astype(np.int64), plan.rot90, plan.keep)
        if self.keep_rec_inputs or plan.lines_mode:
            self.last_rec_batches = []
        if plan.lines_mode:
            return self._decode_groups(plan, launches, want_words, texts)
        for bi, launch in enumerate(launches):
            ids_b = ids[int(starts[bi]): int(starts[bi + 1])]
            if self.keep_rec_inputs:
                self.last_rec_batches.append((ids_b, launch.x, launch.idx, launch.prob))
            launch.done.synchronize()
            if launch.rows is not None:
                t1 = time.perf_counter()
                self._texts_from_rows(launch.rows.numpy(), ids_b, texts)
            else:
                idx_h, prob_h = launch.idx.cpu().numpy(), launch.prob.cpu().numpy()
                t1 = time.perf_counter()
                for i, (t, s) in zip(ids_b.tolist(), ocr_host.ctc_decode(idx_h, prob_h, self.characters)):
                    texts[i] = (t, ocr_host.format_score(s))
            t_dec += time.perf_counter() - t1
        self.stats["t_decode_ms"] = t_dec * 1e3
        return texts

    @staticmethod
    def _scatter_texts(texts, src_of, page_of, n_img, perm=None):
        if perm is not None:
            inv = np.argsort(perm, kind="stable")
            texts = [texts[i] for i in inv.tolist()]
            src_of, page_of = src_of[inv], page_of[inv]
        out = [[[] for _ in range(k)] for k in n_img]
        for t, si, pi in zip(texts, src_of.tolist(), page_of.tolist()):
            out[si][pi].append(t)
        return out

    def boxes_from_maps(self, maps_host: np.ndarray, page_hw: Tuple[int, int], box_thresh: float = 0.3,
                        unclip_ratio: float = 1.8) -> List[np.ndarray]:
        P = maps_host.shape[0]
        res = ocr_host.db_postprocess(maps_host, [page_hw] * P, thresh=0.3, box_thresh=box_thresh, unclip_ratio=unclip_ratio,
                                      raw=self.host_native)
        t0 = time.perf_counter()
        if self.host_native:
            out = ocr_host.order_merge_boxes_native(*res)
            self.stats["t_boxes_ms"] = (time.perf_counter() - t0) * 1e3
            return out
        out = []
        for boxes, _scores in res:
            if len(boxes) == 0:
                out.append(np.zeros((0, 4, 2), np.float32))
                continue
            b = ocr_host.sorted_boxes(boxes.astype(np.float32))
            b = ocr_host.merge_det_boxes(b)
            out.append(np.asarray(b, dtype=np.float32).reshape(-1, 4, 2))
        self.stats["t_boxes_ms"] = (time.perf_counter() - t0) * 1e3
        return out

    def boxes_from_maps_device(self, maps_dev: torch.Tensor, page_hw: Tuple[int, int], box_thresh: float = 0.3,
                               unclip_ratio: float = 1.8) -> List[np.ndarray]:
        P = maps_dev.shape[0]
        res = ocr_host.db_postprocess_device(maps_dev, [page_hw] * P, thresh=0.3, box_thresh=box_thresh, unclip_ratio=unclip_ratio,
                                             stats=self.stats, cache=self.db_ws, raw=self.host_native)
        t0 = time.perf_counter()
        if self.host_native:
            out = ocr_host.order_merge_boxes_native(*res)
            self.stats["t_boxes_ms"] = (time.perf_counter() - t0) * 1e3
            return out
        out = []
        for boxes, _scores in res:
            if len(boxes) == 0:
                out.append(np.zeros((0, 4, 2), np.float32))
                continue
            b = ocr_host.merge_det_boxes(ocr_host.sorted_boxes(boxes.astype(np.float32)))
            out.append(np.asarray(b, dtype=np.float32).reshape(-1, 4, 2))
        self.stats["t_boxes_ms"] = (time.perf_counter() - t0) * 1e3
        return out

    def _boxes_via_host_maps(self, src: torch.Tensor, page_hw: Tuple[int, int]) -> List[np.ndarray]:
        if getattr(self, "_maps_host", None) is None or self._maps_host.shape != src.shape:
            self._maps_host = torch.empty(src.shape, dtype=torch.float32, pin_memory=True)
        t0 = time.perf_counter()
        self._maps_host.copy_(src, non_blocking=True)
        torch.cuda.current_stream().synchronize()
        t1 = time.perf_counter()
        quads = self.boxes_from_maps(self._maps_host.numpy(), page_hw)
        self.stats["t_wait_maps_ms"] = (t1 - t0) * 1e3
        self.stats["t_db_post_ms"] = (time.perf_counter() - t1) * 1e3 - self.stats["t_boxes_ms"]
        return quads

    def run_batch(self, pages: torch.Tensor, quads_per_page: Optional[Sequence[np.ndarray]] = None,
                  det_maps_override: Optional[torch.Tensor] = None, prefetch: Optional[torch.Tensor] = None,
                  page_keys: Optional[Sequence[int]] = None) -> List[PageResult]:
        if isinstance(pages, np.ndarray) or not pages.is_cuda:
            src = torch.from_numpy(np.ascontiguousarray(pages)) if isinstance(pages, np.ndarray) else pages.contiguous()
            pages = src.to(self.tdev, non_blocking=src.is_pinned())
        self._page_keys = None if page_keys is None else [int(k) for k in page_keys]
        assert self._page_keys is None or len(self._page_keys) == pages.shape[0]
        if self.rec_width_sync is not None and page_keys is None and getattr(self.rec_width_sync, "world_size", 1) > 1:
            raise ValueError("rec_width_sync over more than one rank needs page_keys: the pages' positions in the GLOBAL page list")
        self._width_sync_epoch += 1
        self._in_run_batch = True
        try:
            return self._run_batch_guarded(pages, quads_per_page, det_maps_override, prefetch)
        finally:
            self._in_run_batch = False

    def _run_batch_guarded(self, pages, quads_per_page, det_maps_override, prefetch):
        results = self._run_batch_once(pages, quads_per_page, det_maps_override, prefetch)
        engines = [self.det] + ([self.layout] if self.layout is not None else [])
        if os.environ.get("RD_DEV_SKIP_RANGE_CHECK") == "1":
            engines = []
        if any([e.check_range_and_fallback() for e in engines]):
            self.stats["range_fallbacks"] = self.stats.get("range_fallbacks", 0) + 1
            self._prefetched = None
            results = self._run_batch_once(pages, quads_per_page, det_maps_override, prefetch)
        return results

    @staticmethod
    def _front_key(pages: torch.Tensor) -> tuple:
        return (pages.data_ptr(), tuple(pages.shape))

    def _front(self, pages: torch.Tensor, n_results: int, gate: Sequence[torch.cuda.Event] = ()) -> dict:
        cur = torch.cuda.current_stream()
        h = {"key": self._front_key(pages), "feats": None, "layout_done": None}
        self.front_stream.wait_stream(cur)
        for ev in gate:
            self.front_stream.wait_event(ev)
        with torch.cuda.stream(self.front_stream):
            h["prob_maps"], h["det_hw"] = self.det_forward(pages)
            h["det_done"] = torch.cuda.Event()
            h["det_done"].record(self.front_stream)
        if self.layout is not None:
            self.layout_stream.wait_event(h["det_done"])
            with torch.cuda.stream(self.layout_stream):
                feats = self.layout_forward(pages)
                if self.keep_feats:
                    h["feats"] = [[f[i].clone() for f in feats] for i in range(n_results)]
                h["layout_done"] = torch.cuda.Event()
                h["layout_done"].record(self.layout_stream)
        return h

    def _run_batch_once(self, pages: torch.Tensor, quads_per_page: Optional[Sequence[np.ndarray]] = None,
                        det_maps_override: Optional[torch.Tensor] = None, prefetch: Optional[torch.Tensor] = None) -> List[PageResult]:
        assert pages.is_cuda and pages.dtype == torch.uint8 and pages.dim() == 4
        P, H, W, _ = pages.shape
        results = [PageResult() for _ in range(P)]
        cur = torch.cuda.current_stream()
        h, self._prefetched = self._prefetched, None
        if h is None or h["key"] != self._front_key(pages):
            h = self._front(pages, P)
            self.stats["front_prefetched"] = 0.0
        else:
            self.stats["front_prefetched"] = 1.0
        cur.wait_event(h["det_done"])
        if self.rec_width_sync is not None and self.det.precision != "fp32" and os.environ.get("RD_DEV_SKIP_RANGE_CHECK") != "1":
            if self.det.check_range_and_fallback():
                self.stats["range_fallbacks"] = self.stats.get("range_fallbacks", 0) + 1
                h = self._front(pages, P)
                self.stats["front_prefetched"] = 0.0
                cur.wait_event(h["det_done"])
        prob_maps, det_hw = h["prob_maps"], h["det_hw"]
        self.last_det = (prob_maps, det_hw)
        if quads_per_page is None:
            src = det_maps_override if det_maps_override is not None else prob_maps
            quads_per_page = self.boxes_from_maps_device(src.contiguous(), (H, W)) if self.device_db else self._boxes_via_host_maps(src, (H, W))
        if prefetch is not None:
            assert prefetch.is_cuda and prefetch.dtype == torch.uint8 and prefetch.dim() == 4

            def front_next(gate):
                self._prefetched = self._front(prefetch, prefetch.shape[0], gate)
            self._after_rec_enqueue = front_next
        try:
            keys = getattr(self, "_page_keys", None)
            texts = self.rec_forward_sources([(pages, quads_per_page)], image_keys=None if keys is None else [keys])[0]
        except BaseException:
            self._after_rec_enqueue = None
            raise
        if self._after_rec_enqueue is not None:
            self._after_rec_enqueue = None
            front_next(())
        if h["layout_done"] is not None:
            cur.wait_event(h["layout_done"])
        for i in range(P):
            qs = np.asarray(quads_per_page[i], dtype=np.float32).reshape(-1, 4, 2)
            results[i].lines = [(qs[j], t, s) for j, (t, s) in enumerate(texts[i])]
            if h["feats"] is not None:
                results[i].layout_feats = h["feats"][i]
            if self.use_cls and self.last_cls is not None:
                results[i].cls = list(self.last_cls[0][i])
        return results


def render_text_maps(boxes_per_page: Sequence[np.ndarray], page_hw: Tuple[int, int], map_hw: Tuple[int, int],
                     device) -> torch.Tensor:
    H, W = page_hw
    h, w = map_hw
    maps = torch.full((len(boxes_per_page), 1, h, w), 0.02, dtype=torch.float32)
    for i, boxes in enumerate(boxes_per_page):
        for x0, y0, x1, y1 in np.asarray(boxes, dtype=np.float64).reshape(-1, 4):
            bw, bh = x1 - x0, y1 - y0
            d = 0.32 * min(bw, bh)
            xa, xb = int(round((x0 + d) * w / W)), int(round((x1 - d) * w / W))
            ya, yb = int(round((y0 + d) * h / H)), int(round((y1 - d) * h / H))
            if xb > xa and yb > ya:
                maps[i, 0, ya:yb, xa:xb] = 0.9
    return maps.to(device)


class PageUploader:

    def __init__(self, device: int = 0, n_buffers: int = 2):
        self.tdev = torch.device("cuda", device)
        self.stream = torch.cuda.Stream(device=self.tdev)
        self.n = max(2, n_buffers)
        self._dev: List[Optional[torch.Tensor]] = [None] * self.n
        self._pin: List[Optional[torch.Tensor]] = [None] * self.n
        self._released: List[Optional[torch.cuda.Event]] = [None] * self.n
        self._consumer: List[Optional[torch.cuda.Stream]] = [None] * self.n
        self._i = 0
        self.bytes_uploaded = 0

    @staticmethod
    def pinned_like(shape) -> torch.Tensor:
        return torch.empty(tuple(shape), dtype=torch.uint8, pin_memory=True)

    def submit(self, pages_host) -> Tuple[torch.Tensor, torch.cuda.Event, int]:
        src = torch.from_numpy(pages_host) if isinstance(pages_host, np.ndarray) else pages_host
        assert not src.is_cuda and src.dtype == torch.uint8 and src.dim() == 4 and src.is_contiguous()
        k = self._i % self.n
        self._i += 1
        if self._dev[k] is None or self._dev[k].numel() < src.numel():
            self._dev[k] = torch.empty(int(src.numel() * 1.1) + 256, dtype=torch.uint8, device=self.tdev)
        dst = self._dev[k][: src.numel()].view(src.shape)
        if self._consumer[k] is not None:
            rel = torch.cuda.Event()
            rel.record(self._consumer[k])
            self._released[k], self._consumer[k] = rel, None
        if self._released[k] is not None:
            self.stream.wait_event(self._released[k])
        if not src.is_pinned():
            if self._pin[k] is None or self._pin[k].numel() < src.numel():
                self._pin[k] = torch.empty(int(src.numel() * 1.1) + 256, dtype=torch.uint8, pin_memory=True)
            self.stream.synchronize()
            stage = self._pin[k][: src.numel()].view(src.shape)
            stage.copy_(src)
            src = stage
        with torch.cuda.stream(self.stream):
            dst.copy_(src, non_blocking=True)
            ev = torch.cuda.Event()
            ev.record(self.stream)
        self.bytes_uploaded += src.numel()
        return dst, ev, k

    def wait(self, ticket: Tuple[torch.Tensor, torch.cuda.Event, int]) -> torch.Tensor:
        dst, ev, k = ticket
        cur = torch.cuda.current_stream()
        cur.wait_event(ev)
        self._consumer[k] = cur
        return dst

    def release(self, ticket) -> None:
        _dst, _ev, k = ticket
        rel = torch.cuda.Event()
        rel.record(torch.cuda.current_stream())
        self._released[k], self._consumer[k] = rel, None


class PagePipelinePool:

    def __init__(self, states: Dict[str, object], device: int = 0, workers: int = 2, **kw):
        self.device = device
        self.pipes = [PagePipeline(states, device, **kw) for _ in range(max(1, workers))]
        self.streams = [torch.cuda.Stream(device=self.pipes[0].tdev) for _ in self.pipes]
        self.pool = ThreadPoolExecutor(max_workers=len(self.pipes))
        self.stats: Dict[str, float] = {}

    @property
    def engines(self) -> List[RdEngine]:
        out = []
        for p in self.pipes:
            out += [p.det, *([p.layout] if p.layout is not None else []), *p.rec_engines, p.rec_tail]
        return out

    def run_batch(self, pages: torch.Tensor, quads_per_page: Optional[Sequence[np.ndarray]] = None,
                  det_maps_override: Optional[torch.Tensor] = None, prefetch: Optional[torch.Tensor] = None,
                  page_keys: Optional[Sequence[int]] = None) -> List[PageResult]:
        assert page_keys is None or len(self.pipes) == 1 or all(p.rec_width_sync is None for p in self.pipes)
        if isinstance(pages, np.ndarray) or not pages.is_cuda:
            src = torch.from_numpy(np.ascontiguousarray(pages)) if isinstance(pages, np.ndarray) else pages.contiguous()
            pages = src.to(self.pipes[0].tdev, non_blocking=src.is_pinned())
        P = pages.shape[0]
        n = min(len(self.pipes), max(1, P))
        bounds = [P * k // n for k in range(n + 1)]
        nb = None
        if prefetch is not None and min(len(self.pipes), max(1, prefetch.shape[0])) == n:
            nb = [prefetch.shape[0] * k // n for k in range(n + 1)]
        ready = torch.cuda.Event()
        ready.record()

        def work(k: int):
            lo, hi = bounds[k], bounds[k + 1]
            torch.cuda.set_device(self.device)
            st = self.streams[k]
            with torch.cuda.stream(st):
                st.wait_event(ready)
                res = self.pipes[k].run_batch(pages[lo:hi], None if quads_per_page is None else quads_per_page[lo:hi],
                                              None if det_maps_override is None else det_maps_override[lo:hi],
                                              None if nb is None else prefetch[nb[k]:nb[k + 1]],
                                              None if page_keys is None else page_keys[lo:hi])
                done = torch.cuda.Event()
                done.record(st)
            return res, done

        outs = list(self.pool.map(work, range(n)))
        results: List[PageResult] = []
        for res, done in outs:
            torch.cuda.current_stream().wait_event(done)
            results += res
        self.stats = {}
        for k, p in enumerate(self.pipes[:n]):
            for key, v in p.stats.items():
                self.stats[key] = self.stats.get(key, 0.0) + v
        return results
```

### rapiddoc_amd/rec_plan.py

```python
from __future__ import annotations

from dataclasses import dataclass
from typing import Callable, List, Optional, Sequence, Tuple

import numpy as np

from . import ocr_host
from .engine import pad_tail_lengths, rec_line_table

CLS_IMG_H, CLS_IMG_W = 48, 192

LINE_DTYPE = np.dtype([("page", "<i4"), ("out_w", "<i4"), ("crop_w", "<i4"), ("crop_h", "<i4"), ("rot90", "<i4"),
                       ("scratch_off", "<i4"), ("m", "<f8", (9,))])
assert LINE_DTYPE.itemsize == 96


def quad_to_crop_matrix(quad: np.ndarray) -> Tuple[np.ndarray, float, float]:
    q = np.asarray(quad, dtype=np.float64).reshape(4, 2)
    cw = max(np.linalg.norm(q[0] - q[1]), np.linalg.norm(q[2] - q[3]))
    ch = max(np.linalg.norm(q[0] - q[3]), np.linalg.norm(q[1] - q[2]))
    cw, ch = float(int(cw)), float(int(ch))
    cw, ch = max(cw, 1.0), max(ch, 1.0)
    src = np.array([[0, 0], [cw, 0], [cw, ch], [0, ch]], dtype=np.float64)
    A, b = [], []
    for (x, y), (u, v) in zip(src, q):
        A.append([x, y, 1, 0, 0, 0, -u * x, -u * y]); b.append(u)
        A.append([0, 0, 0, x, y, 1, -v * x, -v * y]); b.append(v)
    h = np.linalg.solve(np.asarray(A), np.asarray(b))
    return np.append(h, 1.0).astype(np.float32), cw, ch


def quads_to_crop_matrices(quads: np.ndarray) -> Tuple[np.ndarray, np.ndarray, np.ndarray, np.ndarray]:
    q32 = np.asarray(quads, dtype=np.float32).reshape(-1, 4, 2)
    q = q32.astype(np.float64)
    n = len(q)

    def norm32(a, b):
        d = a - b
        return np.sqrt(d[:, 0] * d[:, 0] + d[:, 1] * d[:, 1])
    cw = np.maximum(norm32(q32[:, 0], q32[:, 1]), norm32(q32[:, 2], q32[:, 3])).astype(np.float64)
    ch = np.maximum(norm32(q32[:, 0], q32[:, 3]), norm32(q32[:, 1], q32[:, 2])).astype(np.float64)
    cw, ch = np.floor(cw), np.floor(ch)
    ok = (cw >= 1.0) & (ch >= 1.0) & np.isfinite(cw) & np.isfinite(ch)
    cw, ch = np.where(ok, cw, 1.0), np.where(ok, ch, 1.0)
    z = np.zeros(n)
    src = np.stack([np.stack([z, z], 1), np.stack([cw, z], 1), np.stack([cw, ch], 1), np.stack([z, ch], 1)], axis=1)
    A = np.zeros((n, 8, 8))
    b = np.zeros((n, 8))
    x, y, u, v = src[..., 0], src[..., 1], q[..., 0], q[..., 1]
    A[:, 0::2, 0], A[:, 0::2, 1], A[:, 0::2, 2] = x, y, 1.0
    A[:, 0::2, 6], A[:, 0::2, 7] = -u * x, -u * y
    A[:, 1::2, 3], A[:, 1::2, 4], A[:, 1::2, 5] = x, y, 1.0
    A[:, 1::2, 6], A[:, 1::2, 7] = -v * x, -v * y
    b[:, 0::2], b[:, 1::2] = u, v
    with np.errstate(all="ignore"):
        for i, j, k in ((0, 1, 2), (1, 2, 3), (2, 3, 0), (3, 0, 1)):
            cross = (q[:, j, 0] - q[:, i, 0]) * (q[:, k, 1] - q[:, i, 1]) - (q[:, j, 1] - q[:, i, 1]) * (q[:, k, 0] - q[:, i, 0])
            ok &= np.isfinite(cross) & (np.abs(cross) > 1e-6 * cw * ch)
    A[~ok] = np.eye(8)
    h = np.linalg.solve(A, b[..., None])[..., 0]
    return np.concatenate([h, np.ones((n, 1))], axis=1), cw, ch, ok


@dataclass
class RecPlan:
    n_img: List[int]
    src_of: np.ndarray
    page_of: np.ndarray
    perm: Optional[np.ndarray]
    keep: np.ndarray
    n_all: int
    lines_mode: bool = False
    two_stage: bool = False
    lines_in_launch: bool = False
    crop_w: Optional[np.ndarray] = None
    crop_h: Optional[np.ndarray] = None
    rot90: Optional[np.ndarray] = None
    eff_w: Optional[np.ndarray] = None
    eff_h: Optional[np.ndarray] = None
    ratios: Optional[List[float]] = None
    order_all: Optional[np.ndarray] = None
    line_ids: Optional[np.ndarray] = None
    line_w: Optional[np.ndarray] = None
    line_ratio: Optional[np.ndarray] = None
    batches: Optional[List[Tuple[np.ndarray, int]]] = None
    starts: Optional[np.ndarray] = None
    descs: Optional[np.ndarray] = None
    descs_cls: Optional[np.ndarray] = None
    descs_warp: Optional[np.ndarray] = None
    warp_jobs: Optional[List[List[Tuple[int, int, int, int]]]] = None
    batch_base: Optional[np.ndarray] = None
    seq_line: Optional[np.ndarray] = None
    groups: Optional[List[List[int]]] = None
    group_lens: Optional[List[np.ndarray]] = None
    group_pad: Optional[List[Tuple[np.ndarray, int]]] = None
    group_base: Optional[np.ndarray] = None
    first_tok: Optional[np.ndarray] = None
    tok_lo: Optional[List[int]] = None
    linetab: Optional[np.ndarray] = None

    @property
    def n(self) -> int:
        return len(self.keep)

    @property
    def scratch_bytes(self) -> int:
        return int(self.batch_base[-1])


def _no_lines(sync, **pooling) -> RecPlan:
    if sync is not None:
        sync(np.zeros(0, np.int64), np.zeros(0))
    return RecPlan(**pooling)


def plan_rec(sources: Sequence[Tuple[int, Sequence[np.ndarray]]], image_keys: Optional[Sequence[Sequence[int]]] = None, *,
             strict: bool, two_stage: bool, lines_in_launch: bool, chunking: str, rec_batch_num: int, rec_width_multiple: int,
             n_cu: int, n_streams: int, use_cls: bool = False, host_native: bool = True, want_words: bool = False,
             width_sync: Optional[Callable] = None) -> RecPlan:
    z32 = np.zeros(0, np.int32)
    n_img = [int(k) for k, _q in sources]
    src_of, page_of, quad_list = [], [], []
    for si, (_k, quads_per_img) in enumerate(sources):
        for pi, q in enumerate(quads_per_img):
            q = np.asarray(q, dtype=np.float64).reshape(-1, 4, 2)
            if len(q):
                quad_list.append(q)
                src_of.append(np.full(len(q), si, np.int32))
                page_of.append(np.full(len(q), pi, np.int32))
    if not quad_list:
        return _no_lines(width_sync, n_img=n_img, src_of=z32, page_of=z32, perm=None, keep=np.zeros(0, np.int64), n_all=0)
    quads = np.concatenate(quad_list, axis=0)
    src_of, page_of = np.concatenate(src_of), np.concatenate(page_of)
    perm = None
    if image_keys is not None:
        key = np.array([image_keys[si][pi] for si, pi in zip(src_of.tolist(), page_of.tolist())], dtype=np.int64)
        perm = np.argsort(key, kind="stable")
        quads, src_of, page_of, key = quads[perm], src_of[perm], page_of[perm], key[perm]
    mats, cws_a, chs_a, ok = quads_to_crop_matrices(quads)
    keep = np.nonzero(ok)[0]
    n = len(keep)
    pooling = dict(n_img=n_img, src_of=src_of, page_of=page_of, perm=perm, keep=keep, n_all=len(quads))
    if n == 0:
        return _no_lines(width_sync, **pooling)
    mats, cws_a, chs_a = mats[keep], cws_a[keep], chs_a[keep]
    rots_a = (chs_a / cws_a >= 2.0).astype(np.int32)
    eff_w = np.where(rots_a == 1, chs_a, cws_a)
    eff_h = np.where(rots_a == 1, cws_a, chs_a)
    ratios = (eff_w / eff_h).tolist()
    lines_mode = strict and two_stage
    if want_words and not lines_mode:
        raise RuntimeError("word boxes need the strict two-stage recogniser (rec_mode='strict', RD_REC_TWO_STAGE unset)")
    line_ratio = None
    if lines_mode:
        given = None
        if width_sync is not None:
            line_keys = key[keep] if image_keys is not None else page_of[keep].astype(np.int64)
            given = width_sync(line_keys, np.asarray(ratios, dtype=np.float64))
        batches, line_w, line_ratio = ocr_host.rec_batches_lines(ratios, n_cu=n_cu, with_ratio=True, given=given, native=host_native)
        if not lines_in_launch:
            batches = ocr_host.rec_batches_equal_width(np.concatenate([c for c, _w in batches]), line_w)
    elif not strict and chunking == "adaptive":
        batches = ocr_host.rec_batches_adaptive(ratios, width_multiple=rec_width_multiple, n_cu=n_cu)
    else:
        batches = ocr_host.rec_batches(ratios, rec_batch_num, width_multiple=rec_width_multiple, strict=strict, merge_equal_width=strict)
    order_all = np.concatenate([c for c, _ in batches])
    if not lines_mode:
        line_w = np.concatenate([np.full(len(c), w) for c, w in batches])
    descs = np.zeros(n, dtype=LINE_DTYPE)
    descs["page"] = page_of[keep][order_all]
    descs["out_w"] = np.minimum(line_w, np.ceil(ocr_host.REC_IMG_H * (eff_w / eff_h)[order_all])).astype(np.int32)
    descs["crop_w"] = cws_a[order_all].astype(np.int32)
    descs["crop_h"] = chs_a[order_all].astype(np.int32)
    descs["m"] = mats[order_all]
    descs["rot90"] = rots_a[order_all]
    crop_bytes = (descs["crop_w"].astype(np.int64) * descs["crop_h"] * 3 + 15) // 16 * 16
    nb = len(batches)
    starts = np.cumsum([0] + [len(c) for c, _ in batches])
    offs = np.zeros(n, np.int64)
    batch_scratch = []
    for b in range(nb):
        cb = crop_bytes[starts[b]:starts[b + 1]]
        offs[starts[b]:starts[b + 1]] = np.cumsum(cb) - cb
        batch_scratch.append(int(cb.sum()))
    if max(batch_scratch) >= 2 ** 31:
        raise RuntimeError("a rec batch needs >= 2 GB of crop scratch: lower rec_batch_num")
    descs["scratch_off"] = offs.astype(np.int32)
    plan = RecPlan(**pooling, lines_mode=lines_mode, two_stage=two_stage, lines_in_launch=lines_mode and lines_in_launch,
                   crop_w=cws_a, crop_h=chs_a, rot90=rots_a, eff_w=eff_w, eff_h=eff_h, ratios=ratios,
                   order_all=order_all, line_ids=keep[order_all], line_w=line_w, line_ratio=line_ratio, batches=batches, starts=starts,
                   descs=descs, batch_base=np.cumsum([0] + batch_scratch))
    crop_px = descs["crop_w"].astype(np.int64) * descs["crop_h"]
    plan.warp_jobs = []
    if len(sources) > 1:
        src_sorted = src_of[keep][order_all]
        warp_order = np.concatenate([starts[b] + np.argsort(src_sorted[starts[b]:starts[b + 1]], kind="stable") for b in range(nb)])
        plan.descs_warp = descs[warp_order]
        ws_sorted = src_sorted[warp_order]
        px_sorted = crop_px[warp_order]
        for b in range(nb):
            lo, hi = int(starts[b]), int(starts[b + 1])
            cuts = [lo] + [i for i in range(lo + 1, hi) if ws_sorted[i] != ws_sorted[i - 1]] + [hi]
            plan.warp_jobs.append([(int(ws_sorted[a]), a, e - a, int(px_sorted[a:e].max())) for a, e in zip(cuts[:-1], cuts[1:])])
    else:
        for b in range(nb):
            lo, hi = int(starts[b]), int(starts[b + 1])
            plan.warp_jobs.append([(0, lo, hi - lo, int(crop_px[lo:hi].max()))])
    if use_cls:
        plan.descs_cls = descs.copy()
        plan.descs_cls["out_w"] = np.minimum(CLS_IMG_W, np.ceil(CLS_IMG_H * (eff_w / eff_h)[order_all])).astype(np.int32)
    if two_stage:
        _plan_tokens(plan, n_streams)
    return plan


def _plan_tokens(plan: RecPlan, S: int) -> None:
    starts, nb = plan.starts, len(plan.batches)
    w2_ = (np.asarray(plan.line_w, dtype=np.int64) - 1) // 2 + 1
    seq_line = ((w2_ - 1) // 2 + 1) // 2
    groups = [list(range(g, min(g + S, nb))) for g in range(0, nb, S)]
    plan.group_lens = [seq_line[int(starts[grp[0]]): int(starts[grp[-1] + 1])] for grp in groups]
    plan.group_pad = [pad_tail_lengths(l) for l in plan.group_lens]
    plan.group_base = np.cumsum([0] + [int(lp.sum()) for lp, _t in plan.group_pad])
    first_tok = np.zeros(plan.n, np.int64)
    for gi, grp in enumerate(groups):
        lo, hi = int(starts[grp[0]]), int(starts[grp[-1] + 1])
        first_tok[lo:hi] = int(plan.group_base[gi]) + np.cumsum(seq_line[lo:hi]) - seq_line[lo:hi]
    plan.seq_line, plan.groups, plan.first_tok = seq_line, groups, first_tok
    plan.tok_lo = [int(first_tok[int(starts[bi])]) for bi in range(nb)]
    if plan.lines_in_launch:
        plan.linetab = rec_line_table(plan.line_w, first_tok)
```

Before: 374.8.

## Build rec plan tables natively in a single staged arena

Moves rec plan construction (line descriptors, warp jobs, token groups, tail padding tables, line table) from numpy loops into a C++ routine that writes everything into one contiguous host arena laid out for a single upload. It also adds a native CTC row scatter and a batched range-zeroing helper. The aim is to cut Python host overhead per page and reduce the number of separate uploads, at the cost of duplicated planning logic that has to match the Python path exactly.

```diff
diff --git a/include/rapiddoc_mi355.h b/include/rapiddoc_mi355.h
--- a/include/rapiddoc_mi355.h
+++ b/include/rapiddoc_mi355.h
@@ -115,6 +115,8 @@
                           float* kept_conf_dev, void* stream);
 int rd_ctc_rows_text(const uint8_t* rows_host, int n, int row_bytes, uint8_t* text_out, int64_t text_cap, int64_t* byte_off_out,
                      int32_t* n_chars_out, double* conf_out, double* conf3_out);
+int rd_ctc_rows_scatter(const uint8_t* rows_host, int n, int row_bytes, const int64_t* line_ids, const int64_t* perm, int64_t n_all,
+                        uint8_t* store, int64_t text_cap, int64_t* used, int64_t* char_off, int32_t* n_chars, double* conf3);
 
 typedef struct rd_text_box {
     float pts[8];
@@ -173,6 +175,19 @@
 int rd_rec_plan_lines(const double* ratios, const int64_t* order, int n, int rec_batch_num, int img_h, int img_w, int launch_multiple,
                       int n_min, int n_max, int n_step, int n_cu, int64_t* line_w_out, double* line_ratio_out, int32_t* sizes_out,
                       int32_t* launch_w_out, int max_out, int32_t* n_out);
+#define RD_PLAN_USE_CLS 1
+#define RD_PLAN_TWO_STAGE 2
+#define RD_PLAN_LINE_TABLE 4
+enum {
+    RD_PLAN_NEED_BYTES = 0, RD_PLAN_UPLOAD_BYTES, RD_PLAN_N_GROUPS, RD_PLAN_N_JOBS, RD_PLAN_N_LINES_PAD, RD_PLAN_MAX_TAIL, RD_PLAN_OFF_LINE_TABLE,
+    RD_PLAN_OFF_TAIL_TABLES, RD_PLAN_OFF_DESCS, RD_PLAN_OFF_DESCS_CLS, RD_PLAN_OFF_DESCS_WARP, RD_PLAN_OFF_STARTS, RD_PLAN_OFF_BATCH_BASE,
+    RD_PLAN_OFF_JOB_START, RD_PLAN_OFF_JOBS, RD_PLAN_OFF_SEQ_LINE, RD_PLAN_OFF_FIRST_TOK, RD_PLAN_OFF_TOK_LO, RD_PLAN_OFF_GROUP_BASE,
+    RD_PLAN_OFF_GROUP_T, RD_PLAN_OFF_PAD_OFF, RD_PLAN_OFF_LENS_PAD, RD_PLAN_OFF_TAIL_OFF, RD_PLAN_OFF_ZERO_RANGES, RD_PLAN_LAYOUT_LEN
+};
+int rd_rec_plan_fill(const double* mats, const double* crop_w, const double* crop_h, const int32_t* page, const int32_t* src, int n,
+                     const int64_t* order, const int64_t* line_w, const int32_t* sizes, int nb, int n_streams, int n_sources, int flags,
+                     int line_cap, int64_t tail_slot, uint8_t* arena, int64_t arena_bytes, int64_t* layout_out);
+int rd_zero_ranges(int device_id, void* base_dev, const int64_t* ranges_host, int n, int64_t unit_bytes, void* stream);
 
 int rd_set_precision(rd_handle* h, const char* mode);
 int rd_range_status(rd_handle* h, void* stream);
diff --git a/rapiddoc_amd/_lib.py b/rapiddoc_amd/_lib.py
--- a/rapiddoc_amd/_lib.py
+++ b/rapiddoc_amd/_lib.py
@@ -50,8 +50,11 @@
     "rd_rec_chunk_cost": (C.c_double, [C.c_int, C.c_int, C.c_int]),
     "rd_rec_plan_chunks": (C.c_int, [C.c_void_p, C.c_int, C.c_int, C.c_int, C.c_int, C.c_int, C.c_void_p, C.c_int, C.c_void_p]),
     "rd_rec_plan_lines": (C.c_int, [C.c_void_p, C.c_void_p] + [C.c_int] * 9 + [C.c_void_p] * 4 + [C.c_int, C.c_void_p]),
+    "rd_rec_plan_fill": (C.c_int, [C.c_void_p] * 5 + [C.c_int, C.c_void_p, C.c_void_p, C.c_void_p] + [C.c_int] * 5 + [C.c_int64, C.c_void_p, C.c_int64, C.c_void_p]),
+    "rd_zero_ranges": (C.c_int, [C.c_int, C.c_void_p, C.c_void_p, C.c_int, C.c_int64, C.c_void_p]),
     "rd_text_boxes_order_merge": (C.c_int, [C.c_void_p, C.c_void_p, C.c_int, C.c_int, C.c_void_p, C.c_void_p]),
     "rd_ctc_rows_text": (C.c_int, [C.c_void_p, C.c_int, C.c_int, C.c_void_p, C.c_int64, C.c_void_p, C.c_void_p, C.c_void_p, C.c_void_p]),
+    "rd_ctc_rows_scatter": (C.c_int, [C.c_void_p, C.c_int, C.c_int, C.c_void_p, C.c_void_p, C.c_int64, C.c_void_p, C.c_int64] + [C.c_void_p] * 4),
     "rd_layout_postprocess": (C.c_int, [C.c_void_p, C.c_int, C.c_int, C.c_int, C.c_int, C.c_void_p, C.c_void_p, C.c_void_p, C.c_void_p]),
     "rd_layout_postprocess_select": (C.c_int, [C.c_void_p, C.c_int, C.c_int, C.c_int, C.c_int, C.c_void_p, C.c_void_p, C.c_void_p, C.c_void_p]),
     "rd_find_external_contours": (C.c_int, [C.c_void_p, C.c_int, C.c_int, C.c_void_p, C.c_int, C.c_void_p, C.c_int, C.c_void_p, C.c_void_p]),
diff --git a/rapiddoc_amd/build.py b/rapiddoc_amd/build.py
--- a/rapiddoc_amd/build.py
+++ b/rapiddoc_amd/build.py
@@ -10,7 +10,7 @@
 PKG = Path(__file__).resolve().parent
 CSRC = PKG / "csrc"
 OUT = PKG / "librapiddoc_mi355.so"
-SOURCES = ["kernels_conv.hip", "kernels_conv_h3.hip", "kernels_conv_direct_h3.hip", "kernels_conv3x3_h1.hip", "kernels_conv9x9_h1.hip", "kernels_stem34.hip", "kernels_rtdetr.hip", "kernels_conv_stream_h3.hip", "kernels_gemm_h3_dma.hip", "kernels_gemm_h1.hip", "kernels_misc.hip", "kernels_dw_lds.hip", "kernels_stem_fused.hip", "kernels_image.hip", "kernels_resize_aa.hip", "kernels_dbpost.hip", "kernels_attention_h3.hip", "kernels_seqconv.hip", "kernels_det_local.hip", "kernels_lcv3.hip", "kernels_lcv3_det.hip", "kernels_mv1e.hip", "kernels_mbv3.hip", "kernels_mbv3s.hip", "kernels_vit_attn.hip", "kernels_lcv3_block.hip", "kernels_ctc.hip", "kernels_mixer.hip", "kernels_mixer_h3.hip", "kernels_mixer_ws.hip", "kernels_mixer_res.hip", "formula_decoder.hip", "table_decoder.hip", "engine.cpp", "builder.cpp", "builder_mobile.cpp", "models.cpp", "api.cpp", "api_debug.cpp", "db_postprocess.cpp", "layout_postprocess.cpp", "polygon_ops.cpp", "rec_chunks.cpp", "host_stages.cpp"]
+SOURCES = ["kernels_conv.hip", "kernels_conv_h3.hip", "kernels_conv_direct_h3.hip", "kernels_conv3x3_h1.hip", "kernels_conv9x9_h1.hip", "kernels_stem34.hip", "kernels_rtdetr.hip", "kernels_conv_stream_h3.hip", "kernels_gemm_h3_dma.hip", "kernels_gemm_h1.hip", "kernels_misc.hip", "kernels_dw_lds.hip", "kernels_stem_fused.hip", "kernels_image.hip", "kernels_resize_aa.hip", "kernels_dbpost.hip", "kernels_attention_h3.hip", "kernels_seqconv.hip", "kernels_det_local.hip", "kernels_lcv3.hip", "kernels_lcv3_det.hip", "kernels_mv1e.hip", "kernels_mbv3.hip", "kernels_mbv3s.hip", "kernels_vit_attn.hip", "kernels_lcv3_block.hip", "kernels_ctc.hip", "kernels_mixer.hip", "kernels_mixer_h3.hip", "kernels_mixer_ws.hip", "kernels_mixer_res.hip", "formula_decoder.hip", "table_decoder.hip", "engine.cpp", "builder.cpp", "builder_mobile.cpp", "models.cpp", "api.cpp", "api_debug.cpp", "db_postprocess.cpp", "layout_postprocess.cpp", "polygon_ops.cpp", "rec_chunks.cpp", "rec_plan_fill.cpp", "host_stages.cpp"]
 FLAGS = ["--offload-arch=gfx950", "-O3", "-std=c++17", "-fPIC", "-Wall", "-Wno-unused-function", "-x", "hip"]
 FILE_FLAGS = {"kernels_mixer_ws.hip": ["-fno-slp-vectorize", "-DRD_GELU_SCALAR"], "kernels_gemm_h1.hip": ["-fno-slp-vectorize"],
               "kernels_stem_fused.hip": ["-fno-slp-vectorize"]}
diff --git a/rapiddoc_amd/csrc/api.cpp b/rapiddoc_amd/csrc/api.cpp
--- a/rapiddoc_amd/csrc/api.cpp
+++ b/rapiddoc_amd/csrc/api.cpp
@@ -298,6 +298,19 @@
     if (hipSetDevice(device_id) != hipSuccess) return 1;
     if (rd::launch_ctc_collapse(idx, prob, B, T, nullptr, ctab, max_len, n_classes, out, row_bytes, nullptr, nullptr, (hipStream_t)stream) != 0) return 1;
     return hipGetLastError() == hipSuccess ? 0 : 1;
+}
+
+int rd_zero_ranges(int device_id, void* base, const int64_t* ranges, int n, int64_t unit_bytes, void* stream) {
+    if (n < 0 || unit_bytes <= 0 || (n > 0 && (!base || !ranges))) return 1;
+    for (int r = 0; r < n; ++r)
+        if (ranges[2 * r] < 0 || ranges[2 * r + 1] < 0) return 1;
+    if (hipSetDevice(device_id) != hipSuccess) return 1;
+    for (int r = 0; r < n; ++r) {
+        if (ranges[2 * r + 1] == 0) continue;
+        if (hipMemsetAsync((uint8_t*)base + ranges[2 * r] * unit_bytes, 0, (size_t)(ranges[2 * r + 1] * unit_bytes), (hipStream_t)stream) != hipSuccess)
+            return 1;
+    }
+    return 0;
 }
 
 int rd_ctc_collapse_lines(int device_id, const int32_t* idx, const float* prob, int n_lines, const int32_t* seg, int max_tokens,
diff --git a/rapiddoc_amd/csrc/host_stages.cpp b/rapiddoc_amd/csrc/host_stages.cpp
--- a/rapiddoc_amd/csrc/host_stages.cpp
+++ b/rapiddoc_amd/csrc/host_stages.cpp
@@ -86,6 +86,14 @@
     return n;
 }
 
+double score_3_decimals(double s) {
+    char buf[400];
+    const auto w = std::to_chars(buf, buf + sizeof(buf), s, std::chars_format::fixed, 3);
+    double r = s;
+    if (w.ec == std::errc()) std::from_chars(buf, w.ptr, r);
+    return r;
+}
+
 }
 
 extern "C" int rd_text_boxes_order_merge(const rd_text_box* boxes, const int32_t* counts, int B, int max_in, float* quads_out, int32_t* n_out) {
@@ -119,13 +127,46 @@
         pos += nbytes;
         byte_off_out[b + 1] = pos;
         n_chars_out[b] = chars;
-        const double s = (double)conf;
-        conf_out[b] = s;
-        char buf[400];
-        const auto w = std::to_chars(buf, buf + sizeof(buf), s, std::chars_format::fixed, 3);
-        double r = s;
-        if (w.ec == std::errc()) std::from_chars(buf, w.ptr, r);
-        conf3_out[b] = r;
+        conf_out[b] = (double)conf;
+        conf3_out[b] = score_3_decimals((double)conf);
     }
     return 0;
 }
+
+extern "C" int rd_ctc_rows_scatter(const uint8_t* rows, int n, int row_bytes, const int64_t* line_ids, const int64_t* perm, int64_t n_all,
+                                   uint8_t* store, int64_t text_cap, int64_t* used, int64_t* char_off, int32_t* n_chars, double* conf3) {
+    if (n < 0 || row_bytes < 16 || text_cap < 0 || n_all < 0 || !used || used[0] < 0 || used[0] > text_cap || used[1] < 0 ||
+        (n > 0 && (!rows || !line_ids || !char_off || !n_chars || !conf3)))
+        return 1;
+    int64_t total = 0;
+    for (int b = 0; b < n; ++b) {
+        int32_t nbytes;
+        std::memcpy(&nbytes, rows + (size_t)b * row_bytes, 4);
+        if (nbytes < 0 || nbytes > row_bytes - 16 || line_ids[b] < 0 || line_ids[b] >= n_all) return 1;
+        if (perm && (perm[line_ids[b]] < 0 || perm[line_ids[b]] >= n_all)) return 1;
+        total += nbytes;
+    }
+    if (used[0] + total > text_cap || (total > 0 && !store)) return 2;
+    int64_t pos = used[0], chars_before = used[1];
+    for (int b = 0; b < n; ++b) {
+        const uint8_t* row = rows + (size_t)b * row_bytes;
+        int32_t nbytes;
+        float conf;
+        std::memcpy(&nbytes, row, 4);
+        std::memcpy(&conf, row + 4, 4);
+        int32_t chars = 0;
+        for (int32_t i = 0; i < nbytes; ++i) {
+            const uint8_t c = row[16 + i];
+            store[pos + i] = c;
+            chars += (c & 0xC0) != 0x80;
+        }
+        pos += nbytes;
+        const int64_t p = perm ? perm[line_ids[b]] : line_ids[b];
+        char_off[p] = chars_before;
+        n_chars[p] = chars;
+        conf3[p] = score_3_decimals((double)conf);
+        chars_before += chars;
+    }
+    used[0] = pos, used[1] = chars_before;
+    return 0;
+}
diff --git a/rapiddoc_amd/csrc/rec_plan_fill.cpp b/rapiddoc_amd/csrc/rec_plan_fill.cpp
--- /dev/null
+++ b/rapiddoc_amd/csrc/rec_plan_fill.cpp
@@ -0,0 +1,253 @@
+#include <algorithm>
+#include <cmath>
+#include <cstdint>
+#include <cstring>
+#include <numeric>
+#include <vector>
+
+#include "../../include/rapiddoc_mi355.h"
+
+#pragma clang fp contract(off)
+
+namespace {
+
+struct LineDesc {
+    int32_t page, out_w, crop_w, crop_h, rot90, scratch_off;
+    double m[9];
+};
+static_assert(sizeof(LineDesc) == 96, "LINE_DTYPE is 96 bytes");
+
+constexpr int64_t TAIL_LINE_BUCKET = 32, TAIL_T_BUCKET = 8, TAIL_TOKEN_BUCKET = 256;
+constexpr int64_t REC_IMG_H = 48, CLS_IMG_H = 48, CLS_IMG_W = 192;
+
+int64_t ceil_to(int64_t v, int64_t m) { return (v + m - 1) / m * m; }
+
+struct Section {
+    int64_t off = -1, bytes = 0;
+};
+
+}
+
+extern "C" int rd_rec_plan_fill(const double* mats, const double* crop_w, const double* crop_h, const int32_t* page, const int32_t* src, int n,
+                                const int64_t* order, const int64_t* line_w, const int32_t* sizes, int nb, int n_streams, int n_sources,
+                                int flags, int line_cap, int64_t tail_slot, uint8_t* arena, int64_t arena_bytes, int64_t* layout_out) {
+    if (!layout_out) return 1;
+    std::fill(layout_out, layout_out + RD_PLAN_LAYOUT_LEN, (int64_t)-1);
+    const bool use_cls = flags & RD_PLAN_USE_CLS, two_stage = flags & RD_PLAN_TWO_STAGE, want_tab = (flags & RD_PLAN_LINE_TABLE) && two_stage;
+    const bool by_source = n_sources > 1;
+    if (n <= 0 || nb <= 0 || n_streams <= 0 || arena_bytes < 0 || line_cap < 0 || tail_slot < 0 || !mats || !crop_w || !crop_h || !page || !order || !line_w || !sizes ||
+        (by_source && !src))
+        return 1;
+    std::vector<int64_t> starts((size_t)nb + 1, 0);
+    for (int b = 0; b < nb; ++b) {
+        if (sizes[b] <= 0) return 1;
+        starts[b + 1] = starts[b] + sizes[b];
+    }
+    if (starts[nb] != n) return 1;
+    for (int j = 0; j < n; ++j) {
+        const int64_t i = order[j];
+        if (i < 0 || i >= n || line_w[j] < 1 || line_w[j] > INT32_MAX) return 1;
+        if (!(crop_w[i] >= 1.0 && crop_w[i] <= 2147483647.0 && crop_h[i] >= 1.0 && crop_h[i] <= 2147483647.0)) return 1;
+        if (by_source && (src[i] < 0 || src[i] >= n_sources)) return 1;
+    }
+
+    const int ng = two_stage ? (nb + n_streams - 1) / n_streams : 0;
+    std::vector<int64_t> seq_line, group_base, group_T, pad_off, lens_pad, tail_off;
+    int64_t max_tail = 0;
+    if (two_stage) {
+        seq_line.resize((size_t)n);
+        for (int j = 0; j < n; ++j) {
+            const int64_t w2 = (line_w[j] - 1) / 2 + 1;
+            seq_line[j] = ((w2 - 1) / 2 + 1) / 2;
+        }
+        group_base.assign((size_t)ng + 1, 0);
+        group_T.resize((size_t)ng);
+        pad_off.assign((size_t)ng + 1, 0);
+        tail_off.assign((size_t)ng + 1, 0);
+        for (int g = 0; g < ng; ++g) {
+            const int64_t lo = starts[(size_t)g * n_streams], hi = starts[std::min<int64_t>((int64_t)(g + 1) * n_streams, nb)];
+            const int64_t cnt = hi - lo;
+            int64_t tok = 0, longest = 0;
+            for (int64_t j = lo; j < hi; ++j) {
+                tok += seq_line[j];
+                longest = std::max(longest, seq_line[j]);
+            }
+            const int64_t T = ceil_to(longest, TAIL_T_BUCKET);
+            if (T <= 0) return 1;
+            int64_t d = (cnt / TAIL_LINE_BUCKET + 1) * TAIL_LINE_BUCKET - cnt, pad;
+            for (;;) {
+                pad = ceil_to(tok + d, TAIL_TOKEN_BUCKET) - tok;
+                if (pad <= d * T) break;
+                d += TAIL_LINE_BUCKET;
+            }
+            const int64_t base = pad / d, extra = pad % d;
+            lens_pad.insert(lens_pad.end(), seq_line.begin() + lo, seq_line.begin() + hi);
+            for (int64_t k = 0; k < d; ++k) lens_pad.push_back(base + (k < extra ? 1 : 0));
+            group_T[g] = T;
+            pad_off[g + 1] = (int64_t)lens_pad.size();
+            group_base[g + 1] = group_base[g] + tok + pad;
+            tail_off[g + 1] = tail_off[g] + 2 * (cnt + d) + tok + pad;
+            max_tail = std::max(max_tail, tail_off[g + 1] - tail_off[g]);
+            if (T >= 32768 || group_base[g + 1] > INT32_MAX) return 1;
+        }
+    }
+
+    const int64_t tab_lines = std::max<int64_t>(line_cap, n);
+    if (two_stage && tail_slot > 0) {
+        tail_slot = std::max(tail_slot, max_tail);
+        for (int g = 0; g <= ng; ++g) tail_off[g] = g * tail_slot;
+    }
+
+    std::vector<int64_t> warp_order;
+    int64_t n_jobs = nb;
+    if (by_source) {
+        warp_order.resize((size_t)n);
+        std::iota(warp_order.begin(), warp_order.end(), (int64_t)0);
+        n_jobs = 0;
+        for (int b = 0; b < nb; ++b) {
+            std::stable_sort(warp_order.begin() + starts[b], warp_order.begin() + starts[b + 1],
+                             [&](int64_t a, int64_t c) { return src[order[a]] < src[order[c]]; });
+            for (int64_t j = starts[b]; j < starts[b + 1]; ++j)
+                n_jobs += j == starts[b] || src[order[warp_order[j]]] != src[order[warp_order[j - 1]]];
+        }
+    }
+
+    int64_t pos = 0;
+    auto take = [&](int64_t bytes) {
+        Section s;
+        s.off = pos;
+        s.bytes = bytes;
+        pos = ceil_to(pos + bytes, 16);
+        return s;
+    };
+    const Section s_tab = want_tab ? take(tab_lines * 16) : Section(), s_tail = two_stage ? take(tail_off[ng] * 4) : Section();
+    const Section s_descs = take((int64_t)n * 96), s_cls = use_cls ? take((int64_t)n * 96) : Section(),
+                  s_warp = by_source ? take((int64_t)n * 96) : Section();
+    const int64_t upload_bytes = pos;
+    const Section s_starts = take((nb + 1) * 8), s_bbase = take((nb + 1) * 8), s_jstart = take((nb + 1) * 8), s_jobs = take(n_jobs * 32);
+    Section s_seq, s_first, s_toklo, s_gbase, s_gT, s_poff, s_lpad, s_toff, s_zero;
+    if (two_stage) {
+        s_seq = take((int64_t)n * 8), s_first = take((int64_t)n * 8), s_toklo = take((int64_t)nb * 8), s_gbase = take((ng + 1) * 8);
+        s_gT = take(ng * 8), s_poff = take((ng + 1) * 8), s_lpad = take((int64_t)lens_pad.size() * 8), s_toff = take((ng + 1) * 8);
+        s_zero = take(ng * 16);
+    }
+    layout_out[RD_PLAN_NEED_BYTES] = pos;
+    if (!arena || arena_bytes < pos) return 2;
+    layout_out[RD_PLAN_UPLOAD_BYTES] = upload_bytes;
+    layout_out[RD_PLAN_N_GROUPS] = ng;
+    layout_out[RD_PLAN_N_JOBS] = n_jobs;
+    layout_out[RD_PLAN_N_LINES_PAD] = (int64_t)lens_pad.size();
+    layout_out[RD_PLAN_MAX_TAIL] = max_tail;
+    layout_out[RD_PLAN_OFF_TAIL_TABLES] = s_tail.off, layout_out[RD_PLAN_OFF_LINE_TABLE] = s_tab.off, layout_out[RD_PLAN_OFF_DESCS] = s_descs.off;
+    layout_out[RD_PLAN_OFF_DESCS_CLS] = s_cls.off, layout_out[RD_PLAN_OFF_DESCS_WARP] = s_warp.off, layout_out[RD_PLAN_OFF_STARTS] = s_starts.off;
+    layout_out[RD_PLAN_OFF_BATCH_BASE] = s_bbase.off, layout_out[RD_PLAN_OFF_JOB_START] = s_jstart.off, layout_out[RD_PLAN_OFF_JOBS] = s_jobs.off;
+    layout_out[RD_PLAN_OFF_SEQ_LINE] = s_seq.off, layout_out[RD_PLAN_OFF_FIRST_TOK] = s_first.off, layout_out[RD_PLAN_OFF_TOK_LO] = s_toklo.off;
+    layout_out[RD_PLAN_OFF_GROUP_BASE] = s_gbase.off, layout_out[RD_PLAN_OFF_GROUP_T] = s_gT.off, layout_out[RD_PLAN_OFF_PAD_OFF] = s_poff.off;
+    layout_out[RD_PLAN_OFF_LENS_PAD] = s_lpad.off, layout_out[RD_PLAN_OFF_TAIL_OFF] = s_toff.off, layout_out[RD_PLAN_OFF_ZERO_RANGES] = s_zero.off;
+    std::memset(arena, 0, (size_t)upload_bytes);
+
+    LineDesc* descs = reinterpret_cast<LineDesc*>(arena + s_descs.off);
+    int64_t* batch_base = reinterpret_cast<int64_t*>(arena + s_bbase.off);
+    std::vector<int64_t> crop_px((size_t)n);
+    std::vector<double> cls_w(use_cls ? (size_t)n : 0);
+    batch_base[0] = 0;
+    bool too_large = false;
+    for (int b = 0; b < nb; ++b) {
+        int64_t off = 0;
+        for (int64_t j = starts[b]; j < starts[b + 1]; ++j) {
+            const int64_t i = order[j];
+            const double cw = crop_w[i], ch = crop_h[i];
+            const bool rot = ch / cw >= 2.0;
+            const double ratio = (rot ? ch : cw) / (rot ? cw : ch);
+            LineDesc& d = descs[j];
+            d.page = page[i];
+            d.out_w = (int32_t)std::min((double)line_w[j], std::ceil((double)REC_IMG_H * ratio));
+            d.crop_w = (int32_t)cw;
+            d.crop_h = (int32_t)ch;
+            d.rot90 = rot ? 1 : 0;
+            d.scratch_off = (int32_t)off;
+            std::memcpy(d.m, mats + 9 * i, sizeof(d.m));
+            crop_px[j] = (int64_t)d.crop_w * d.crop_h;
+            off += (crop_px[j] * 3 + 15) / 16 * 16;
+            if (use_cls) cls_w[j] = std::min((double)CLS_IMG_W, std::ceil((double)CLS_IMG_H * ratio));
+        }
+        too_large |= off >= ((int64_t)1 << 31);
+        batch_base[b + 1] = batch_base[b] + off;
+    }
+    if (too_large) return 3;
+    std::memcpy(arena + s_starts.off, starts.data(), (size_t)(nb + 1) * 8);
+    if (use_cls) {
+        LineDesc* dc = reinterpret_cast<LineDesc*>(arena + s_cls.off);
+        std::memcpy(dc, descs, (size_t)n * 96);
+        for (int j = 0; j < n; ++j) dc[j].out_w = (int32_t)cls_w[j];
+    }
+
+    int64_t* job_start = reinterpret_cast<int64_t*>(arena + s_jstart.off);
+    int64_t* jobs = reinterpret_cast<int64_t*>(arena + s_jobs.off);
+    int64_t nj = 0;
+    job_start[0] = 0;
+    if (by_source) {
+        LineDesc* dw = reinterpret_cast<LineDesc*>(arena + s_warp.off);
+        for (int j = 0; j < n; ++j) dw[j] = descs[warp_order[j]];
+        for (int b = 0; b < nb; ++b) {
+            for (int64_t j = starts[b]; j < starts[b + 1]; ++j) {
+                const int32_t s = src[order[warp_order[j]]];
+                const int64_t px = crop_px[warp_order[j]];
+                if (j == starts[b] || s != (int32_t)jobs[4 * (nj - 1)]) {
+                    jobs[4 * nj] = s, jobs[4 * nj + 1] = j, jobs[4 * nj + 2] = 0, jobs[4 * nj + 3] = px;
+                    ++nj;
+                }
+                jobs[4 * (nj - 1) + 2] += 1;
+                jobs[4 * (nj - 1) + 3] = std::max(jobs[4 * (nj - 1) + 3], px);
+            }
+            job_start[b + 1] = nj;
+        }
+    } else {
+        for (int b = 0; b < nb; ++b) {
+            jobs[4 * nj] = 0, jobs[4 * nj + 1] = starts[b], jobs[4 * nj + 2] = starts[b + 1] - starts[b];
+            jobs[4 * nj + 3] = *std::max_element(crop_px.begin() + starts[b], crop_px.begin() + starts[b + 1]);
+            job_start[b + 1] = ++nj;
+        }
+    }
+    if (nj != n_jobs) return 1;
+    if (!two_stage) return 0;
+
+    int64_t* first_tok = reinterpret_cast<int64_t*>(arena + s_first.off);
+    int64_t* tok_lo = reinterpret_cast<int64_t*>(arena + s_toklo.off);
+    int64_t* zero = reinterpret_cast<int64_t*>(arena + s_zero.off);
+    int32_t* tail = reinterpret_cast<int32_t*>(arena + s_tail.off);
+    for (int g = 0; g < ng; ++g) {
+        const int64_t lo = starts[(size_t)g * n_streams], hi = starts[std::min<int64_t>((int64_t)(g + 1) * n_streams, nb)];
+        int64_t t = group_base[g];
+        for (int64_t j = lo; j < hi; ++j) {
+            first_tok[j] = t;
+            t += seq_line[j];
+        }
+        zero[2 * g] = t, zero[2 * g + 1] = group_base[g + 1] - t;
+        const int64_t L = pad_off[g + 1] - pad_off[g];
+        int32_t* seg = tail + tail_off[g];
+        int32_t* tokinfo = seg + 2 * L;
+        int64_t off = 0;
+        for (int64_t l = 0; l < L; ++l) {
+            const int64_t len = lens_pad[pad_off[g] + l];
+            seg[2 * l] = (int32_t)off, seg[2 * l + 1] = (int32_t)len;
+            for (int64_t p = 0; p < len; ++p) tokinfo[off + p] = (int32_t)(p | (len << 16));
+            off += len;
+        }
+    }
+    for (int b = 0; b < nb; ++b) tok_lo[b] = first_tok[starts[b]];
+    if (want_tab) {
+        int32_t* tab = reinterpret_cast<int32_t*>(arena + s_tab.off);
+        for (int j = 0; j < n; ++j) {
+            const int64_t w = line_w[j], w2 = (w - 1) / 2 + 1, w4 = (w2 - 1) / 2 + 1;
+            tab[4 * j] = (int32_t)w, tab[4 * j + 1] = (int32_t)w2, tab[4 * j + 2] = (int32_t)w4, tab[4 * j + 3] = (int32_t)first_tok[j];
+        }
+    }
+    std::memcpy(arena + s_seq.off, seq_line.data(), (size_t)n * 8);
+    std::memcpy(arena + s_gbase.off, group_base.data(), (size_t)(ng + 1) * 8);
+    std::memcpy(arena + s_gT.off, group_T.data(), (size_t)ng * 8);
+    std::memcpy(arena + s_poff.off, pad_off.data(), (size_t)(ng + 1) * 8);
+    std::memcpy(arena + s_lpad.off, lens_pad.data(), lens_pad.size() * 8);
+    std::memcpy(arena + s_toff.off, tail_off.data(), (size_t)(ng + 1) * 8);
+    return 0;
+}
diff --git a/rapiddoc_amd/pipeline.py b/rapiddoc_amd/pipeline.py
--- a/rapiddoc_amd/pipeline.py
+++ b/rapiddoc_amd/pipeline.py
@@ -12,7 +12,7 @@
 
 from . import _lib, ocr_host
 from .engine import RdEngine, preproc_resize_norm, preproc_resize_norm_batch
-from .rec_plan import (CLS_IMG_H, CLS_IMG_W, LINE_DTYPE, RecPlan, plan_rec,
+from .rec_plan import (CLS_IMG_H, CLS_IMG_W, LINE_DTYPE, PlanStage, RecPlan, plan_rec,
                        quad_to_crop_matrix, quads_to_crop_matrices)
 
 LAYOUT_SIZE = 800
@@ -61,6 +61,74 @@
     cols: Optional[Tuple[torch.Tensor, torch.Tensor]] = None
     cls_prob: Optional[torch.Tensor] = None
     cls_flip: Optional[torch.Tensor] = None
+
+
+class _PinnedStage(PlanStage):
+    sticky = True
+
+    def __init__(self):
+        self._bufs: List[Optional[torch.Tensor]] = [None, None]
+        self._sent: List[Optional[torch.cuda.Event]] = [None, None]
+        self._i = 0
+
+    def turn(self) -> None:
+        self._i ^= 1
+        if self._sent[self._i] is not None:
+            self._sent[self._i].synchronize()
+
+    def get(self, n_bytes: int) -> np.ndarray:
+        t = self._bufs[self._i]
+        if t is None or t.numel() < n_bytes:
+            t = self._bufs[self._i] = torch.empty(max(int(n_bytes * 1.5), 1 << 20), dtype=torch.uint8, pin_memory=True)
+        return t.numpy()
+
+    def upload(self, dst: torch.Tensor) -> None:
+        dst.copy_(self._bufs[self._i][: dst.numel()], non_blocking=True)
+        if self._sent[self._i] is None:
+            self._sent[self._i] = torch.cuda.Event()
+        self._sent[self._i].record(torch.cuda.current_stream())
+
+
+class _PageTexts:
+
+    def __init__(self, lib, n_all: int, perm: Optional[np.ndarray]):
+        self._lib, self.n_all = lib, int(n_all)
+        self._perm = None if perm is None else np.ascontiguousarray(perm, dtype=np.int64)
+        self._store = np.empty(max(64 * self.n_all, 4096), np.uint8)
+        self._used = np.zeros(2, np.int64)
+        self._char_off, self._n_chars, self._conf3 = np.zeros(self.n_all, np.int64), np.zeros(self.n_all, np.int32), np.zeros(self.n_all)
+        self._text = np.full(self.n_all, "", dtype=object)
+
+    def add(self, rows_np: np.ndarray, line_ids: np.ndarray) -> None:
+        rows, ids = np.ascontiguousarray(rows_np), np.ascontiguousarray(line_ids, dtype=np.int64)
+        n, row_bytes = rows.shape
+        b0, c0 = self._used.tolist()
+        need = b0 + n * max(0, row_bytes - 16)
+        if need > len(self._store):
+            grown = np.empty(2 * need, np.uint8)
+            grown[:b0] = self._store[:b0]
+            self._store = grown
+        rc = self._lib.rd_ctc_rows_scatter(rows.ctypes.data, n, row_bytes, ids.ctypes.data, None if self._perm is None else self._perm.ctypes.data,
+                                           self.n_all, self._store.ctypes.data, len(self._store), self._used.ctypes.data,
+                                           self._char_off.ctypes.data, self._n_chars.ctypes.data, self._conf3.ctypes.data)
+        if rc != 0:
+            raise RuntimeError("rd_ctc_rows_scatter failed")
+        s = self._store[b0: int(self._used[0])].tobytes().decode("utf-8")
+        at = ids if self._perm is None else self._perm[ids]
+        self._text[at] = [s[a: a + k] for a, k in zip((self._char_off[at] - c0).tolist(), self._n_chars[at].tolist())]
+
+    def lines(self) -> List[Tuple[str, float]]:
+        return list(zip(self._text.tolist(), self._conf3.tolist()))
+
+    def pages(self, lines_per_img: Sequence[Sequence[int]]) -> List[List[List[Tuple[str, float]]]]:
+        flat, out, pos = self.lines(), [], 0
+        for counts in lines_per_img:
+            out.append([])
+            for k in counts:
+                out[-1].append(flat[pos: pos + k])
+                pos += k
+        assert pos == self.n_all
+        return out
 
 
 class PagePipeline:
@@ -123,6 +191,7 @@
         self.device_ctc = True
         self.device_db = True
         self.host_native = ocr_host.host_native_default()
+        self._stage = _PinnedStage()
         self.db_ws: dict = {}
         self.rec_two_stage = os.environ.get("RD_REC_TWO_STAGE", "1") != "0"
         self.rec_width_sync = None
@@ -235,10 +304,13 @@
         sync = None
         if self.rec_width_sync is not None and strict and self.rec_two_stage and self._sync_this_call:
             sync = lambda keys, ratios: self._synced_widths(self.rec_width_sync, keys, ratios)
+        if self.host_native:
+            self._stage.turn()
         plan = plan_rec([(imgs.shape[0], quads) for imgs, quads in sources], image_keys, strict=strict, two_stage=self.rec_two_stage,
                         lines_in_launch=self.rec_lines_in_launch, chunking=self.rec_chunking, rec_batch_num=self.rec_batch_num,
                         rec_width_multiple=self.rec_width_multiple, n_cu=self.n_cu, n_streams=len(self.rec_engines), use_cls=self.use_cls,
-                        host_native=self.host_native, want_words=want_words, width_sync=sync)
+                        host_native=self.host_native, want_words=want_words, width_sync=sync,
+                        stage=self._stage if self.host_native else None, stats=self.stats)
         scatter = lambda per_line: self._scatter_texts(per_line, plan.src_of, plan.page_of, plan.n_img, plan.perm)
         cls_of: List[tuple] = [(False, 0, 0.0)] * plan.n_all
         if plan.n == 0:
@@ -272,20 +344,31 @@
                 cls_of[i] = (bool(fh[j]), label, float(ph[j, label]))
             self.last_cls = scatter(cls_of)
             self.last_cls_prob = (plan.line_ids, ph)
-        return scatter(texts)
+        t1 = time.perf_counter()
+        out = texts.pages(plan.lines_per_img) if isinstance(texts, _PageTexts) else scatter(texts)
+        self.stats["t_scatter_ms"] = (time.perf_counter() - t1) * 1e3
+        return out
 
     def _enqueue_rec(self, plan: RecPlan, sources, want_words: bool) -> List[_RecLaunch]:
         dev, S, lib = sources[0][0].device, len(self.rec_engines), self._lib
         keep_inputs = self.keep_rec_inputs
-        upload = lambda descs: torch.from_numpy(descs.view(np.uint8)).to(dev, non_blocking=True)
-        descs_dev = upload(plan.descs)
+        staged = plan.stage is not None
+        if staged:
+            L, n = plan.stage_layout, plan.n
+            stage_dev = self._buf("rec_stage", L["upload_bytes"], torch.uint8)
+            self._stage.upload(stage_dev)
+            upload = lambda descs: stage_dev[L[descs]: L[descs] + n * LINE_DTYPE.itemsize]
+            descs_dev = upload("descs")
+        else:
+            upload = lambda descs: torch.from_numpy(descs.view(np.uint8)).to(dev, non_blocking=True)
+            descs_dev = upload(plan.descs)
         cls = None
         if self.use_cls:
-            cls = (upload(plan.descs_cls), self._buf("cls_prob", 2 * plan.n).view(plan.n, 2), self._buf("cls_flip", plan.n, torch.int32),
+            cls = (upload("descs_cls" if staged else plan.descs_cls), self._buf("cls_prob", 2 * plan.n).view(plan.n, 2), self._buf("cls_flip", plan.n, torch.int32),
                    torch.empty((plan.n, 2), dtype=torch.float32, pin_memory=True), torch.empty((plan.n,), dtype=torch.int32, pin_memory=True))
-        descs_warp_dev = upload(plan.descs_warp) if plan.descs_warp is not None else descs_dev
+        descs_warp_dev = upload("descs_warp" if staged else plan.descs_warp) if plan.descs_warp is not None else descs_dev
         if keep_inputs:
-            self.last_rec_descs = (plan.descs.copy(), np.asarray(plan.batch_base, dtype=np.int64), np.asarray(plan.starts, dtype=np.int64))
+            self.last_rec_descs = (plan.descs.copy(), np.array(plan.batch_base, dtype=np.int64), np.array(plan.starts, dtype=np.int64))
             self.last_cls_inputs = []
         main = torch.cuda.current_stream()
         ready = torch.cuda.Event()
@@ -294,11 +377,20 @@
         if plan.two_stage:
             base = plan.group_base
             tokens = self._buf("rec_tokens", int(base[-1]) * self.rec.rec_token_dim).view(int(base[-1]), self.rec.rec_token_dim)
-            for gi, lens in enumerate(plan.group_lens):
-                tokens[int(base[gi]) + int(lens.sum()): int(base[gi + 1])].zero_()
-            tables = [self.rec_tail.rec_tail_tables(lp, dev, out=self._buf(("tail_tab", gi), 2 * len(lp) + int(lp.sum()), torch.int32))
-                      for gi, (lp, _t) in enumerate(plan.group_pad)]
-            if plan.linetab is not None:
+            if staged:
+                if lib.rd_zero_ranges(self.device, tokens.data_ptr(), plan.zero_ranges.ctypes.data, len(plan.groups),
+                                      4 * self.rec.rec_token_dim, main.cuda_stream) != 0:
+                    raise RuntimeError("rd_zero_ranges failed")
+                t0, off = L["tail_tables"], plan.tail_off.tolist()
+                tables = [stage_dev[t0 + 4 * a: t0 + 4 * e].view(torch.int32) for a, e in zip(off[:-1], off[1:])]
+                if plan.linetab is not None:
+                    linetab = stage_dev[L["line_table"]: L["line_table"] + 16 * n].view(torch.int32).view(n, 4)
+            else:
+                for gi, lens in enumerate(plan.group_lens):
+                    tokens[int(base[gi]) + int(lens.sum()): int(base[gi + 1])].zero_()
+                tables = [self.rec_tail.rec_tail_tables(lp, dev, out=self._buf(("tail_tab", gi), 2 * len(lp) + int(lp.sum()), torch.int32))
+                          for gi, (lp, _t) in enumerate(plan.group_pad)]
+            if plan.linetab is not None and not staged:
                 tab_h = torch.from_numpy(plan.linetab).pin_memory()
                 linetab = self._buf("rec_linetab", 4 * plan.n, torch.int32).view(plan.n, 4)
                 linetab.copy_(tab_h, non_blocking=True)
@@ -395,10 +487,8 @@
             launch.done = done
 
     def _texts_from_rows(self, rows_np: np.ndarray, line_ids: np.ndarray, texts: list) -> None:
-        if self.host_native:
-            txt, _conf, conf3 = ocr_host.parse_ctc_rows_native(rows_np)
-            for i, t, s in zip(line_ids.tolist(), txt, conf3):
-                texts[i] = (t, s)
+        if isinstance(texts, _PageTexts):
+            texts.add(rows_np, line_ids)
         else:
             for i, (t, s) in zip(line_ids.tolist(), ocr_host.parse_ctc_rows(rows_np)):
                 texts[i] = (t, ocr_host.format_score(s))
@@ -438,6 +528,8 @@
 
     def _decode_rec(self, plan: RecPlan, launches: List[_RecLaunch], want_words: bool) -> list:
         texts: List[tuple] = [("", 0.0, None) if want_words else ("", 0.0)] * plan.n_all
+        if self.host_native and self.device_ctc and not want_words:
+            texts = _PageTexts(self._lib, plan.n_all, plan.perm)
         ids, starts = plan.line_ids, plan.starts
         t_dec = 0.0
         if self.keep_rec_inputs:
@@ -622,7 +714,7 @@
             cur.wait_event(h["layout_done"])
         for i in range(P):
             qs = np.asarray(quads_per_page[i], dtype=np.float32).reshape(-1, 4, 2)
-            results[i].lines = [(qs[j], t, s) for j, (t, s) in enumerate(texts[i])]
+            results[i].lines = [(q, t, s) for q, (t, s) in zip(qs, texts[i])]
             if h["feats"] is not None:
                 results[i].layout_feats = h["feats"][i]
             if self.use_cls and self.last_cls is not None:
diff --git a/rapiddoc_amd/rec_plan.py b/rapiddoc_amd/rec_plan.py
--- a/rapiddoc_amd/rec_plan.py
+++ b/rapiddoc_amd/rec_plan.py
@@ -1,11 +1,12 @@
 from __future__ import annotations
 
+import time
 from dataclasses import dataclass
-from typing import Callable, List, Optional, Sequence, Tuple
+from typing import Callable, Dict, List, Optional, Sequence, Tuple
 
 import numpy as np
 
-from . import ocr_host
+from . import _lib, ocr_host
 from .engine import pad_tail_lengths, rec_line_table
 
 CLS_IMG_H, CLS_IMG_W = 48, 192
@@ -98,6 +99,11 @@
     first_tok: Optional[np.ndarray] = None
     tok_lo: Optional[List[int]] = None
     linetab: Optional[np.ndarray] = None
+    lines_per_img: Optional[List[List[int]]] = None
+    stage: Optional[np.ndarray] = None
+    stage_layout: Optional[Dict[str, int]] = None
+    tail_off: Optional[np.ndarray] = None
+    zero_ranges: Optional[np.ndarray] = None
 
     @property
     def n(self) -> int:
@@ -117,19 +123,23 @@
 def plan_rec(sources: Sequence[Tuple[int, Sequence[np.ndarray]]], image_keys: Optional[Sequence[Sequence[int]]] = None, *,
              strict: bool, two_stage: bool, lines_in_launch: bool, chunking: str, rec_batch_num: int, rec_width_multiple: int,
              n_cu: int, n_streams: int, use_cls: bool = False, host_native: bool = True, want_words: bool = False,
-             width_sync: Optional[Callable] = None) -> RecPlan:
+             width_sync: Optional[Callable] = None, stage: Optional["PlanStage"] = None,
+             stats: Optional[dict] = None) -> RecPlan:
     z32 = np.zeros(0, np.int32)
     n_img = [int(k) for k, _q in sources]
     src_of, page_of, quad_list = [], [], []
+    lines_per_img: List[List[int]] = [[0] * k for k in n_img]
     for si, (_k, quads_per_img) in enumerate(sources):
         for pi, q in enumerate(quads_per_img):
             q = np.asarray(q, dtype=np.float64).reshape(-1, 4, 2)
+            lines_per_img[si][pi] = len(q)
             if len(q):
                 quad_list.append(q)
                 src_of.append(np.full(len(q), si, np.int32))
                 page_of.append(np.full(len(q), pi, np.int32))
     if not quad_list:
-        return _no_lines(width_sync, n_img=n_img, src_of=z32, page_of=z32, perm=None, keep=np.zeros(0, np.int64), n_all=0)
+        return _no_lines(width_sync, n_img=n_img, src_of=z32, page_of=z32, perm=None, keep=np.zeros(0, np.int64), n_all=0,
+                         lines_per_img=lines_per_img)
     quads = np.concatenate(quad_list, axis=0)
     src_of, page_of = np.concatenate(src_of), np.concatenate(page_of)
     perm = None
@@ -140,7 +150,7 @@
     mats, cws_a, chs_a, ok = quads_to_crop_matrices(quads)
     keep = np.nonzero(ok)[0]
     n = len(keep)
-    pooling = dict(n_img=n_img, src_of=src_of, page_of=page_of, perm=perm, keep=keep, n_all=len(quads))
+    pooling = dict(n_img=n_img, src_of=src_of, page_of=page_of, perm=perm, keep=keep, n_all=len(quads), lines_per_img=lines_per_img)
     if n == 0:
         return _no_lines(width_sync, **pooling)
     mats, cws_a, chs_a = mats[keep], cws_a[keep], chs_a[keep]
@@ -167,6 +177,15 @@
     order_all = np.concatenate([c for c, _ in batches])
     if not lines_mode:
         line_w = np.concatenate([np.full(len(c), w) for c, w in batches])
+    if host_native:
+        t0 = time.perf_counter()
+        plan = RecPlan(**pooling, lines_mode=lines_mode, two_stage=two_stage, lines_in_launch=lines_mode and lines_in_launch,
+                       crop_w=cws_a, crop_h=chs_a, rot90=rots_a, eff_w=eff_w, eff_h=eff_h, ratios=ratios,
+                       order_all=order_all, line_ids=keep[order_all], line_w=line_w, line_ratio=line_ratio, batches=batches)
+        _fill_native(plan, mats, page_of[keep], src_of[keep], len(sources), n_streams, use_cls, stage)
+        if stats is not None:
+            stats["t_plan_native_ms"] = (time.perf_counter() - t0) * 1e3
+        return plan
     descs = np.zeros(n, dtype=LINE_DTYPE)
     descs["page"] = page_of[keep][order_all]
     descs["out_w"] = np.minimum(line_w, np.ceil(ocr_host.REC_IMG_H * (eff_w / eff_h)[order_all])).astype(np.int32)
@@ -214,6 +233,79 @@
     return plan
 
 
+PLAN_LAYOUT = ("need_bytes", "upload_bytes", "n_groups", "n_jobs", "n_lines_pad", "max_tail", "line_table", "tail_tables", "descs", "descs_cls", "descs_warp",
+               "starts", "batch_base", "job_start", "jobs", "seq_line", "first_tok", "tok_lo", "group_base", "group_T", "pad_off", "lens_pad",
+               "tail_off", "zero_ranges")
+PLAN_COUNTS = PLAN_LAYOUT[:6]
+PLAN_USE_CLS, PLAN_TWO_STAGE, PLAN_LINE_TABLE = 1, 2, 4
+
+
+class PlanStage:
+    line_cap, tail_slot, sticky = 0, 0, False
+
+    def get(self, n_bytes: int) -> np.ndarray:
+        return np.empty(max(int(n_bytes), 1 << 20), np.uint8)
+
+    def fit(self, lines: int, tail_elems: int) -> None:
+        if self.sticky and lines > self.line_cap:
+            self.line_cap = int(lines * 1.25) + 64
+        if self.sticky and tail_elems > self.tail_slot:
+            self.tail_slot = (int(tail_elems * 1.25) + 1024) // 4 * 4
+
+
+def _fill_native(plan: RecPlan, mats: np.ndarray, page_kept: np.ndarray, src_kept: np.ndarray, n_sources: int, S: int, use_cls: bool,
+                 stage: Optional["PlanStage"]) -> None:
+    if stage is None:
+        stage = PlanStage()
+    lib = _lib.load()
+    n, nb = plan.n, len(plan.batches)
+    mats, cw, ch = (np.ascontiguousarray(a, dtype=np.float64) for a in (mats, plan.crop_w, plan.crop_h))
+    page, src = np.ascontiguousarray(page_kept, dtype=np.int32), np.ascontiguousarray(src_kept, dtype=np.int32)
+    order, line_w = np.ascontiguousarray(plan.order_all, dtype=np.int64), np.ascontiguousarray(plan.line_w, dtype=np.int64)
+    sizes = np.array([len(c) for c, _w in plan.batches], dtype=np.int32)
+    flags = (PLAN_USE_CLS if use_cls else 0) | (PLAN_TWO_STAGE if plan.two_stage else 0) | (PLAN_LINE_TABLE if plan.lines_in_launch else 0)
+    layout = np.empty(len(PLAN_LAYOUT), np.int64)
+    stage.fit(n, 0)
+    buf = stage.get(0)
+    for _ in range(2):
+        assert buf.dtype == np.uint8 and buf.ndim == 1 and buf.flags.c_contiguous
+        rc = lib.rd_rec_plan_fill(mats.ctypes.data, cw.ctypes.data, ch.ctypes.data, page.ctypes.data, src.ctypes.data, n, order.ctypes.data,
+                                  line_w.ctypes.data, sizes.ctypes.data, nb, int(S), int(n_sources), flags, int(stage.line_cap), int(stage.tail_slot),
+                                  buf.ctypes.data, buf.nbytes, layout.ctypes.data)
+        if rc != 2:
+            break
+        buf = stage.get(int(layout[0]))
+    if rc == 3:
+        raise RuntimeError("a rec batch needs >= 2 GB of crop scratch: lower rec_batch_num")
+    if rc != 0:
+        raise RuntimeError("rd_rec_plan_fill failed")
+    L = dict(zip(PLAN_LAYOUT, layout.tolist()))
+    stage.fit(n, L["max_tail"])
+
+    def view(key, dtype, count):
+        return buf[L[key]: L[key] + count * np.dtype(dtype).itemsize].view(dtype)
+    plan.stage, plan.stage_layout = buf, L
+    plan.starts, plan.batch_base = view("starts", np.int64, nb + 1), view("batch_base", np.int64, nb + 1)
+    plan.descs = view("descs", LINE_DTYPE, n)
+    plan.descs_cls = view("descs_cls", LINE_DTYPE, n) if use_cls else None
+    plan.descs_warp = view("descs_warp", LINE_DTYPE, n) if n_sources > 1 else None
+    jobs, job_start = view("jobs", np.int64, 4 * L["n_jobs"]).reshape(-1, 4).tolist(), view("job_start", np.int64, nb + 1).tolist()
+    plan.warp_jobs = [[tuple(j) for j in jobs[a:e]] for a, e in zip(job_start[:-1], job_start[1:])]
+    if not plan.two_stage:
+        return
+    ng = L["n_groups"]
+    plan.seq_line, plan.first_tok = view("seq_line", np.int64, n), view("first_tok", np.int64, n)
+    plan.tok_lo = view("tok_lo", np.int64, nb).tolist()
+    plan.group_base, plan.tail_off = view("group_base", np.int64, ng + 1), view("tail_off", np.int64, ng + 1)
+    plan.zero_ranges = view("zero_ranges", np.int64, 2 * ng)
+    plan.groups = [list(range(g, min(g + S, nb))) for g in range(0, nb, S)]
+    starts, pad_off, lens_pad = plan.starts.tolist(), view("pad_off", np.int64, ng + 1).tolist(), view("lens_pad", np.int64, L["n_lines_pad"])
+    plan.group_lens = [plan.seq_line[starts[grp[0]]: starts[grp[-1] + 1]] for grp in plan.groups]
+    plan.group_pad = [(lens_pad[a:e], T) for a, e, T in zip(pad_off[:-1], pad_off[1:], view("group_T", np.int64, ng).tolist())]
+    if plan.lines_in_launch:
+        plan.linetab = view("line_table", np.int32, 4 * n).reshape(n, 4)
+
+
 def _plan_tokens(plan: RecPlan, S: int) -> None:
     starts, nb = plan.starts, len(plan.batches)
     w2_ = (np.asarray(plan.line_w, dtype=np.int64) - 1) // 2 + 1
```

Result: faster. 381.3, median of 5 (+1.7%).
